# iwbn/flow-supervisor

Measured on AMD Instinct MI355X. Metric: image-pairs/s fwd+bwd, 12 GRU iters, 436x1024, higher is better.
Workload: dtype f32 (bf16x3 products); 1 GPU; RAFT full, 440x1024 (Sintel 436x1024 padded), 12 GRU iters, 4 pairs/GPU, train step = fwd + sequence loss + bwd + RCCL all-reduce + clip + AdamW; global_batch=4, parallelism=dp1, launch=hipGraph replay of the whole step

## Files before the change

### flow_supervisor_amd/_lib.py

```python
import ctypes
import functools
import os
from ctypes import POINTER, Structure, c_double, c_float, c_int, c_int64, c_void_p

import torch

_HERE = os.path.dirname(os.path.abspath(__file__))
LIB_PATH = os.environ.get("FSRAFT_LIB_PATH") or os.path.join(_HERE, "libfsraft.so")
_lib = None

c_float_p = c_void_p


class ConvDesc(Structure):
    _fields_ = [
        ("src", c_void_p * 3), ("srcC", c_int * 3), ("srcld", c_int * 3), ("nsrc", c_int),
        ("wpk", c_void_p), ("bias", c_void_p), ("wpk_split", c_void_p),
        ("B", c_int), ("H", c_int), ("W", c_int), ("KH", c_int), ("KW", c_int), ("N", c_int),
        ("dst", c_void_p * 3), ("dst_bs", c_int64 * 3), ("dst_ps", c_int64 * 3), ("dst_cs", c_int64 * 3),
        ("dst_n0", c_int * 3), ("dst_acc", c_int * 3), ("ndst", c_int),
        ("relu", c_int), ("alpha", c_float),
        ("epi", c_int),
        ("h", c_void_p), ("ldh", c_int), ("z", c_void_p), ("ldz", c_int),
        ("aux1", c_void_p), ("ld1", c_int), ("aux2", c_void_p), ("ld2", c_int), ("hid", c_int),
        ("pre", c_void_p), ("ldpre", c_int),
        ("rmask", c_void_p * 3), ("ldmask", c_int * 3), ("maskc", c_int * 3),
        ("wpk_frag", c_void_p), ("pad_h1", c_int), ("pad_w1", c_int),
        ("ws", c_void_p), ("ws_floats", c_int64),
    ]


class PackJob(Structure):
    _fields_ = [
        ("w", c_void_p * 3), ("rows", c_int * 3), ("npiece", c_int),
        ("wpk", c_void_p),
        ("cin_full", c_int), ("kh", c_int), ("kw", c_int),
        ("srcC", c_int * 3), ("srcOff", c_int * 3), ("nsrc", c_int),
        ("mode", c_int), ("flags", c_int),
        ("scale", c_float), ("accumulate", c_int),
    ]


class AugParams(Structure):
    _fields_ = [
        ("resize", c_int), ("th", c_int), ("tw", c_int),
        ("scale_x", c_float), ("scale_y", c_float),
        ("win_y", c_int), ("win_x", c_int), ("hflip", c_int), ("vflip", c_int), ("crop_y", c_int), ("crop_x", c_int),
        ("asym", c_int),
        ("brightness", c_float * 2), ("contrast", c_float * 2), ("saturation", c_float * 2), ("hue", c_float * 2),
        ("nrect", c_int),
        ("rect", (c_int * 4) * 2),
    ]


_PP = POINTER(c_void_p)
_IP = POINTER(c_int)
_S = c_void_p

SIGNATURES = {
    "fsraft_corr_build": [c_void_p, c_void_p, _PP, c_int, c_int, c_int, c_int, c_int, _S],
    "fsraft_corr_unpool_bwd": [_PP, c_int, c_int, c_int, c_int, _S],
    "fsraft_corr_lookup_fwd": [_PP, c_int, c_void_p, c_int64, c_int64, c_int64, c_void_p, c_int, c_int, c_int, c_int, c_int, _S],
    "fsraft_corr_lookup_bwd": [_PP, c_int, c_void_p, c_int64, c_int64, c_int64, c_void_p, c_int, c_int, c_int, c_int, c_int, _S],
    "fsraft_altcorr_fwd": [c_void_p, c_void_p, c_void_p, c_void_p, c_int, c_int, c_int, c_int, c_int, c_int, c_int, c_int, _S],
    "fsraft_altcorr_bwd": [c_void_p, c_void_p, c_void_p, c_void_p, c_void_p, c_void_p, c_int, c_int, c_int, c_int, c_int, c_int, c_int, c_int, _S],
    "fsraft_upsample_fwd": [c_void_p, c_int64, c_int64, c_int64, c_void_p, c_void_p, c_int, c_int, c_int, _S],
    "fsraft_upsample_bwd": [c_void_p, c_int64, c_int64, c_int64, c_void_p, c_void_p, c_void_p, c_void_p, c_void_p, c_int, c_int, c_int, _S],
    "fsraft_upflow8_fwd": [c_void_p, c_void_p, c_int, c_int, c_int, c_int, _S],
    "fsraft_upflow8_bwd": [c_void_p, c_void_p, c_int, c_int, c_int, c_int, _S],
    "fsraft_conv_ktot": [_IP, c_int, c_int, c_int],
    "fsraft_conv_forward": [POINTER(ConvDesc), _S],
    "fsraft_conv_forward_stats": [POINTER(ConvDesc), c_void_p, c_void_p, c_int, POINTER(c_int), _S],
    "fsraft_conv_wgrad": [c_void_p, c_int, c_int, _PP, _IP, _IP, c_int, c_void_p, c_void_p, c_int, c_int, c_int, c_int, c_int, _S],
    "fsraft_conv_wgrad_multi": [_PP, c_int, c_int, c_int, _PP, _IP, _IP, c_int, c_void_p, c_void_p, c_int, c_int, c_int, c_int, c_int, _S],
    "fsraft_conv_small_fwd": [c_void_p, c_int, c_int, c_void_p, c_void_p, c_void_p, c_int64, c_int64, c_int64, c_int, c_int, c_int, c_int, c_int, c_int, _S],
    "fsraft_conv_small_wgrad": [_PP, _PP, c_int, c_int, c_int, c_int, c_void_p, c_void_p, c_int, c_int, c_int, c_int, c_int, c_int, _S],
    "fsraft_conv_small_dgrad": [c_void_p, c_int, c_void_p, c_void_p, c_int, c_void_p, c_int, c_int, c_int, c_int, c_int, c_int, c_int, c_int, _S],
    "fsraft_pack_conv_weights": [POINTER(PackJob), c_int, _S],
    "fsraft_pack_conv_weight": [c_void_p, c_void_p, c_int, c_int, c_int, c_int, _IP, c_int, c_int, c_int, _S],
    "fsraft_set_rec_mfma16": [c_int],
    "fsraft_set_build_kernel": [c_int],
    "fsraft_set_dvol_policy": [c_int],
    "fsraft_set_dvol_box": [c_int],
    "fsraft_set_ktile_exact": [c_int],
    "fsraft_set_lookup_policy": [c_int],
    "fsraft_set_upsample_kernel": [c_int],
    "fsraft_conv_workspace": [c_void_p, c_int64],
    "fsraft_set_arithmetic": [c_int],
    "fsraft_get_arithmetic": [],
    "fsraft_set_tuning": [c_int, c_int],
    "fsraft_adamw_flat": [c_void_p, c_void_p, c_void_p, c_void_p, c_int64, c_void_p, c_void_p, c_float, c_void_p, c_double, c_double, c_float,
                          c_float, c_void_p, c_void_p, _S],
    "fsraft_stream_capture_id": [_S, c_void_p],
    "fsraft_stem_slots": [],
    "fsraft_stem7x7s2_fwd": [c_void_p, c_void_p, c_void_p, c_void_p, c_int, c_int, c_int, c_int, _S],
    "fsraft_stem7x7s2_wgrad": [c_void_p, c_void_p, c_void_p, c_void_p, c_int, c_int, c_int, c_int, _S],
    "fsraft_set_lookup_qb": [c_int],
    "fsraft_set_build_split": [c_int],
    "fsraft_set_gemm_split": [c_int],
    "fsraft_gemm_tn_split": [c_void_p, c_int64, c_int64, c_void_p, c_int64, c_int64, c_void_p, c_int64, c_int64, c_int, c_int, c_int, c_int, c_float, c_int, _S],
    "fsraft_gemm_f32": [c_void_p, c_int64, c_int64, c_void_p, c_int64, c_int64, c_void_p, c_int64, c_int64, c_int, c_int, c_int, c_int, c_int, c_float, c_int, _S],
    "fsraft_nchw_to_nhwc": [c_void_p, c_void_p, c_int, c_int, c_int, c_int, c_int, c_int, _S],
    "fsraft_nhwc_to_nchw": [c_void_p, c_void_p, c_int, c_int, c_int, c_int, c_int, c_int, _S],
    "fsraft_im2col7": [c_void_p, c_int64, c_int64, c_int64, c_void_p, c_int, c_int, c_int, c_int, _S],
    "fsraft_col2im7": [c_void_p, c_int, c_void_p, c_int, c_int, c_int, c_int, _S],
    "fsraft_flow_to_nhwc": [c_void_p, c_int64, c_int64, c_int64, c_void_p, c_int, c_int, c_int, c_int, _S],
    "fsraft_nhwc_to_flow": [c_void_p, c_int, c_int, c_void_p, c_int, c_int, c_int, _S],
    "fsraft_relu_bwd": [c_void_p, c_int, c_void_p, c_int, c_int64, c_int, _S],
    "fsraft_gru_bwd1": [c_void_p, c_void_p, c_void_p, c_void_p, c_void_p, c_void_p, c_int, c_void_p, c_void_p, c_void_p, c_void_p, c_int64, c_int, _S],
    "fsraft_gru_bwd2": [c_void_p, c_void_p, c_void_p, c_void_p, c_int, c_void_p, c_void_p, c_int64, c_int, _S],
    "fsraft_col_sum": [c_void_p, c_int, c_int64, c_int, c_void_p, c_float, _S],
    "fsraft_softmax_rows": [c_void_p, c_int64, c_int, _S],
    "fsraft_softmax_rows_bwd": [c_void_p, c_void_p, c_int64, c_int, _S],
    "fsraft_softmax_rows_rec": [c_void_p, c_int64, c_int, _S],
    "fsraft_softmax_rows_bwd_rec": [c_void_p, c_void_p, c_int64, c_int, _S],
    "fsraft_softmax_rows_pos": [c_void_p, c_void_p, c_int64, c_int64, c_int, c_int, c_int, c_int, c_int, _S],
    "fsraft_softmax_rows_pos_bwd": [c_void_p, c_void_p, c_void_p, c_int64, c_int64, c_int, c_int, c_int, c_int, _S],
    "fsraft_gma_mix_fwd": [c_void_p, c_int, c_void_p, c_int, c_void_p, c_void_p, c_int, c_int64, c_int, _S],
    "fsraft_gma_mix_bwd": [c_void_p, c_int, c_void_p, c_int, c_void_p, c_void_p, c_int, c_void_p, c_int, c_void_p, c_int64, c_int, _S],
    "fsraft_inorm_relu_fwd": [c_void_p, c_void_p, c_void_p, c_int64, c_int, c_float, c_int, _S],
    "fsraft_inorm_relu_bwd": [c_void_p, c_void_p, c_void_p, c_void_p, c_int64, c_int, c_int, _S],
    "fsraft_affine_relu_fwd": [c_void_p, c_void_p, c_void_p, c_void_p, c_int64, c_int, c_int, c_int, _S],
    "fsraft_affine_relu_bwd": [c_void_p, c_void_p, c_void_p, c_void_p, c_void_p, c_void_p, c_void_p, c_int64, c_int, c_int, c_int, _S],
    "fsraft_sequence_loss": [_PP, _PP, POINTER(c_float), c_int, c_int, c_void_p, c_void_p, c_float, c_float, c_int, c_int, c_int, c_void_p, _S],
    "fsraft_flow_loss_workspace_bytes": [c_int, c_int, c_int],
    "fsraft_flow_loss": [_PP, _PP, POINTER(c_float), c_int, c_int64, c_int64, c_int64, c_void_p, c_int64, c_int64, c_int64,
                         c_void_p, c_int64, c_int64, c_int, c_float, c_float, c_float, c_int, c_int, c_int,
                         c_void_p, c_void_p, c_int, c_void_p, c_void_p, c_int64, _S],
    "fsraft_corr_pool_pyramid": [_PP, c_int, c_int64, c_int, c_int, _S],
    "fsraft_corr_pool_pyramid_same": [_PP, c_int, c_int64, c_int, c_int, _S],
    "fsraft_corr_lookup_fwd_same": [_PP, c_int, c_void_p, c_int64, c_int64, c_int64, c_void_p, c_int, c_int, c_int, c_int, c_int, _S],
    "fsraft_corr_unpool_same_bwd": [_PP, c_int, c_int64, c_int, c_int, _S],
    "fsraft_corr_lookup_bwd_same": [_PP, c_int, c_void_p, c_int64, c_int64, c_int64, c_void_p, c_int, c_int, c_int, c_int, c_int, _S],
    "fsraft_corr_lookup_dcoords_same": [_PP, c_int, c_void_p, c_int64, c_int64, c_int64, c_void_p, c_int, c_void_p, c_int64, c_int64, c_int64,
                                        c_int, c_int, c_int, c_int, _S],
    "fsraft_set_norm_blocks": [c_int],
    "fsraft_get_tuning": [c_int],
    "fsraft_conv_last_route": [c_int],
    "fsraft_set_wgrad_wide": [c_int],
    "fsraft_conv_wgrad_last_tile": [],
    "fsraft_space_to_depth2": [c_void_p, c_void_p, c_int, c_int, c_int, c_int, c_int, _S],
    "fsraft_forward_interpolate": [c_void_p, c_void_p, c_int, c_int, _S],
    "fsraft_flow_metrics_scratch_bytes": [c_int, c_int, c_int],
    "fsraft_flow_metrics": [c_void_p, c_int64, c_int64, c_int64, c_void_p, c_int64, c_int64, c_int64, c_void_p, c_int64, c_int64,
                            c_int, c_int, c_int, c_void_p, c_void_p, c_void_p, c_int64, _S],
    "fsraft_flow_rad_max": [c_void_p, c_int64, c_int64, c_int64, c_int, c_int, c_int, c_float, c_void_p, _S],
    "fsraft_flow_wheel": [c_void_p, c_int64, c_int64, c_int64, c_int, c_int, c_int, c_float, c_void_p, c_float, c_int, c_void_p, _S],
    "fsraft_flow_hsv": [c_void_p, c_int64, c_int64, c_int64, c_int, c_int, c_int, c_void_p, c_float, c_int, c_void_p, _S],
    "fsraft_flow_kitti16": [c_void_p, c_int64, c_int64, c_int64, c_void_p, c_int64, c_int64, c_int, c_int, c_int, c_void_p, _S],
    "fsraft_range_map_scratch_bytes": [c_int, c_int, c_int],
    "fsraft_range_map": [c_void_p, c_int64, c_int64, c_int64, c_int, c_int, c_int, c_int, c_void_p, c_void_p, c_int64, _S],
    "fsraft_census_scratch_bytes": [c_int, c_int, c_int],
    "fsraft_census_fwd": [c_void_p, c_int64, c_int64, c_int64, c_int, c_void_p, c_int64, c_int64, c_int64, c_int, c_int, _IP,
                          c_void_p, c_int64, c_int64, c_int64, c_void_p, c_int64, c_int64, c_int, c_int, c_int,
                          c_void_p, c_void_p, c_void_p, c_void_p, c_int64, _S],
    "fsraft_census_bwd": [c_void_p, c_int64, c_int64, c_int64, c_int, c_void_p, c_int64, c_int64, c_int64, c_int, c_int, _IP,
                          c_void_p, c_int64, c_int64, c_int64, c_void_p, c_void_p, c_void_p, c_void_p, c_int, c_int, c_int,
                          c_void_p, _S],
    "fsraft_smoothness_scratch_bytes": [c_int, c_int, c_int],
    "fsraft_smoothness": [c_void_p, c_int64, c_int64, c_int64, c_int, c_int, _IP, c_void_p, c_int64, c_int64, c_int64,
                          c_int, c_int, c_int, c_int, c_float, c_int, c_void_p, c_void_p, c_void_p, c_int64, _S],
    "fsraft_fb_mask": [c_void_p, c_int64, c_int64, c_int64, c_void_p, c_int64, c_int64, c_int64, c_int, c_int, _IP,
                       c_int, c_int, c_int, c_int, c_int, c_float, c_void_p, _S],
    "fsraft_selfsup_scratch_bytes": [c_int, c_int, c_int],
    "fsraft_selfsup": [c_void_p, c_int64, c_int64, c_int64, c_int, c_int, _IP, c_void_p, c_int64, c_int64,
                       c_void_p, c_int64, c_int64, c_int64, c_void_p, c_int64, c_int64, c_int64, c_int, c_int, c_int,
                       c_int, c_float, c_void_p, c_void_p, c_void_p, c_int64, _S],
    "fsraft_augment_scratch_bytes": [c_int, c_int, c_int, c_int, c_int],
    "fsraft_augment": [c_void_p, c_void_p, c_int, c_void_p, c_void_p, c_int, c_int, c_int, POINTER(AugParams), c_int, c_int, c_int, c_int,
                       c_void_p, c_void_p, c_void_p, c_void_p, c_void_p, c_void_p, c_void_p, c_void_p, c_void_p, c_int64, _S],
    "fsraft_augment_sup_scratch_bytes": [c_int, c_int, c_int],
    "fsraft_augment_sup": [c_void_p, c_void_p, c_int, c_void_p, c_void_p, c_int, c_int, c_int, c_int, POINTER(AugParams), c_int, c_int,
                           c_void_p, c_void_p, c_void_p, c_void_p, c_void_p, c_int64, _S],
    "fsraft_inorm_relu_cl_fwd": [c_void_p, c_void_p, c_void_p, c_void_p, c_void_p, c_void_p, c_int, c_int, c_int, c_float, c_int, c_int, c_int, _S],
    "fsraft_inorm_relu_cl_bwd": [c_void_p, c_void_p, c_void_p, c_void_p, c_void_p, c_void_p, c_void_p, c_void_p, c_int, c_int, c_int,
                                 c_int, c_int, _S],
    "fsraft_affine_relu_cl_fwd": [c_void_p, c_void_p, c_void_p, c_void_p, c_void_p, c_int64, c_int, c_int, c_int, c_int, _S],
    "fsraft_affine_relu_cl_bwd": [c_void_p, c_void_p, c_void_p, c_void_p, c_void_p, c_void_p, c_void_p, c_void_p, c_void_p, c_int, c_int,
                                  c_int, c_int, c_int, _S],
    "fsraft_axpby": [c_void_p, c_void_p, c_float, c_float, c_int64, _S],
    "fsraft_sum_n": [_PP, c_int, c_void_p, c_int64, c_int, _S],
    "fsraft_bn_fold": [c_void_p, c_void_p, c_void_p, c_void_p, c_void_p, c_float, c_int, c_void_p, c_void_p, c_void_p, c_void_p, _S],
    "fsraft_bn_fold_bwd": [c_void_p, c_int, c_int, c_void_p, c_void_p, c_void_p, c_void_p, c_void_p, c_void_p, _S],
    "fsraft_bnorm_cl_fwd": [c_void_p, c_void_p, c_void_p, c_void_p, c_void_p, c_void_p, c_void_p, c_float, c_float, c_void_p, c_void_p,
                            c_void_p, c_int, c_int, c_int, c_int, c_int, _S],
    "fsraft_bnorm_cl_bwd": [c_void_p, c_void_p, c_void_p, c_void_p, c_void_p, c_void_p, c_void_p, c_void_p, c_void_p, c_int, c_int,
                            c_int, c_int, c_int, _S],
    "fsraft_vol_layout": [c_int, c_int, c_int, _IP],
    "fsraft_corr_build_tiled": [c_void_p, c_void_p, c_void_p, c_int, c_int, c_int, c_int, c_int, _S],
    "fsraft_corr_build_rec": [c_void_p, c_void_p, c_void_p, c_int, c_int, c_int, c_int, c_int, _S],
    "fsraft_corr_lookup_tiled_fwd": [c_void_p, c_int, c_void_p, c_int64, c_int64, c_int64, c_void_p, c_int, c_int, c_int, c_int, c_int, _S],
    "fsraft_corr_lookup_tiled_dcoords": [c_void_p, c_int, c_void_p, c_int64, c_int64, c_int64, c_void_p, c_void_p, c_int64, c_int64, c_int64,
                                         c_int, c_int, c_int, c_int, c_int, _S],
    "fsraft_corr_lookup_dcoords": [_PP, c_int, c_void_p, c_int64, c_int64, c_int64, c_void_p, c_int, c_void_p, c_int64, c_int64, c_int64,
                                   c_int, c_int, c_int, c_int, _S],
    "fsraft_corr_dvol_build": [_PP, _PP, POINTER(c_int64), c_int, c_void_p, c_int, c_int, c_int, c_int, c_int, c_int, c_int, c_int, c_int64,
                               c_int64, c_void_p, c_void_p, _S],
    "fsraft_set_alt_tile": [c_int],
    "fsraft_altcorr_fused_fwd": [c_void_p, _PP, c_int, c_void_p, c_int64, c_int64, c_int64, c_int, c_void_p, c_int, c_int, c_int, c_int, c_int, _S],
    "fsraft_altcorr_fused_dcoords": [c_void_p, _PP, c_int, c_void_p, c_int64, c_int64, c_int64, c_int, c_void_p, c_void_p, c_int64, c_int64,
                                     c_int64, c_int, c_int, c_int, c_int, c_int, _S],
    "fsraft_altcorr_mfma_fwd": [c_void_p, _PP, c_void_p, _PP, c_int, c_void_p, c_int64, c_int64, c_int64, c_int, c_void_p, c_int, c_int, c_int, c_int, c_int, _S],
    "fsraft_corr_f2cat": [c_void_p, c_void_p, c_int, c_int, c_int, c_int, c_int, _S],
    "fsraft_corr_dfmap2": [c_void_p, c_void_p, c_int, c_int, c_int, c_int, c_int, _S],
    "fsraft_corr_f2cat_rec": [c_void_p, c_void_p, c_int, c_int, c_int, c_int, c_int, _S],
    "fsraft_to_records": [c_void_p, c_int64, c_void_p, c_int64, c_int64, c_int, _S],
    "fsraft_gemm_rec_tn": [c_void_p, c_int64, c_int64, c_void_p, c_int64, c_int64, c_void_p, c_int64, c_int64, c_int, c_int, c_int, c_int,
                           c_float, c_int, c_int, _S],
    "fsraft_gemm_rec_nt": [c_void_p, c_int64, c_int64, c_void_p, c_int64, c_int64, c_void_p, c_int64, c_int64, c_int, c_int, c_int, c_int,
                           c_float, c_int, c_int, _S],
    "fsraft_gemm_rec_nt_list": [c_void_p, c_int64, c_int64, c_void_p, c_int64, c_int64, c_void_p, c_int64, c_int64, c_int, c_int, c_int, c_int,
                                c_float, c_int, c_int, c_void_p, c_void_p, c_int, c_int, _S],
    "fsraft_gemm_rec_tn_list": [c_void_p, c_int64, c_int64, c_void_p, c_int64, c_int64, c_void_p, c_int64, c_int64, c_int, c_int, c_int, c_int,
                                c_float, c_int, c_int, c_void_p, c_void_p, c_int, c_int, _S],
    "fsraft_corr_bwd_ktiles": [_PP, POINTER(c_int64), c_int, c_int, c_int, c_int, c_int, c_int, c_int, c_int64, c_int64, c_void_p, c_void_p,
                               c_int, c_void_p, c_void_p, c_void_p, c_int, c_void_p, _S],
}

CONV_ROUTES = {
    1: ("fwd.gemm32", "fp32"), 2: ("fwd.gemm64", "fp32"), 3: ("fwd.gemm64x128", "fp32"), 4: ("fwd.gemm128", "fp32"),
    5: ("fwd.gemm64x64", "fp32"), 6: ("fwd.gemm64x64k16", "fp32"), 7: ("fwd.gemm64x128k16", "fp32"),
    10: ("fwd.patch128x128", "bf16x3"), 11: ("fwd.patch256x128", "bf16x3"), 12: ("fwd.patch128x64", "bf16x3"),
# ... 110 lines not shown
```

### flow_supervisor_amd/core/extractor.py

```python
import os
from collections import namedtuple

import torch
import torch.nn as nn
import torch.nn.functional as F

from .. import ops
from .._lib import on_tensor_device


class _InstNormRelu(torch.autograd.Function):

    @staticmethod
    def forward(ctx, x, eps, relu):
        x = x.contiguous()
        y, stats = ops.inorm_relu_fwd(x, eps, relu)
        ctx.save_for_backward(x, stats)
        ctx.relu = relu
        return y

    @staticmethod
    def backward(ctx, g):
        x, stats = ctx.saved_tensors
        return ops.inorm_relu_bwd(g.contiguous(), x, stats, ctx.relu), None, None
# ... 309 lines not shown
STATS_IN_EPILOGUE = True
STEM_KERNEL = True
S2D_UNITS = True
TRAIN_BN = True


class _NormSums:
    __slots__ = ("acc",)

    def __init__(self):
        self.acc = None


def _conv(conv, x, bias, link=None, stem_cl=False, sums=None):
    k = conv.kernel_size
    if (_is_cl(x) and x.is_cuda and x.dtype == torch.float32 and k in ((3, 3), (1, 1)) and conv.stride == (1, 1)
            and conv.padding == (k[0] // 2, k[1] // 2) and conv.dilation == (1, 1) and conv.groups == 1
            and conv.padding_mode == "zeros" and x.shape[1] % 4 == 0 and not torch.is_autocast_enabled()):
        return _ConvCL.apply(x, conv.weight, bias, _weight_packs(conv), link, sums)
    if stem_cl and bias is None and _stem_ok(conv, x):
        return _StemFn.apply(x, conv.weight)
    return F.conv2d(_ToNCHW.apply(x) if _is_cl(x) else x, conv.weight, bias, conv.stride, conv.padding, conv.dilation, conv.groups)


_S2D_TAP = ((0, 1), (1, 0), (1, 1))


def _s2d_weight(w3):
    N, C = w3.shape[:2]
    w = w3.new_zeros(N, 2, 2, C, 2, 2)
    for ky, (ty, sy) in enumerate(_S2D_TAP):
        for kx, (tx, sx) in enumerate(_S2D_TAP):
            w[:, sy, sx, :, ty, tx] = w3[:, :, ky, kx]
    return w.reshape(N, 4 * C, 2, 2)


def _s2d_weight_grad(dw, C):
    N = dw.shape[0]
    d = dw.reshape(N, 2, 2, C, 2, 2)
    out = dw.new_empty(N, C, 3, 3)
    for ky, (ty, sy) in enumerate(_S2D_TAP):
        for kx, (tx, sx) in enumerate(_S2D_TAP):
            out[:, :, ky, kx] = d[:, sy, sx, :, ty, tx]
    return out


def _pair_structure_ok(block):
    c1 = getattr(block, "conv1", None)
    ds = block.downsample[0] if getattr(block, "downsample", None) is not None else None
    return (block.n == 2 and c1 is not None and ds is not None and c1.kernel_size == (3, 3) and c1.stride == (2, 2)
            and c1.padding == (1, 1) and c1.dilation == (1, 1) and c1.groups == 1 and ds.kernel_size == (1, 1)
            and ds.stride == (2, 2) and ds.padding == (0, 0) and ds.groups == 1)


def _pair_ok(block, C, H, W):
    return (S2D_UNITS and _pair_structure_ok(block) and H % 2 == 0 and W % 2 == 0 and C % 4 == 0
            and _cl_channels_ok(block.conv1.out_channels))


def _pair_packs(block):
    if _stale(block, "_fs_pair_packs", _pair_key(block)):
        _prepare_packs(block)
    return block.__dict__["_fs_pair_packs"]


class _StridedPairFn(torch.autograd.Function):

    @staticmethod
    def forward(ctx, x, w3, wsc, packs, pre=False):
        x = _as_cl(x)
        ctx.pre = pre
        if pre:
            B, C4, h, w = x.shape
            C, H, W = C4 // 4, 2 * h, 2 * w
            xs = x.permute(0, 2, 3, 1)
        else:
            B, C, H, W = x.shape
            h, w = H // 2, W // 2
            xs = ops.space_to_depth2(x.permute(0, 2, 3, 1))
        N, Ns = w3.shape[0], wsc.shape[0]
        y1 = torch.empty(B, h, w, N, device=x.device, dtype=torch.float32)
        ys = torch.empty(B, h, w, Ns, device=x.device, dtype=torch.float32)
        p, q = packs.conv3, packs.shortcut
        ops.conv_forward([ops.V(xs, 4 * C)], p.fwd, None, B, h, w, 2, 2, N, [ops.Dst.nhwc(y1)], wpk_split=p.fwd_split)
        ops.conv_forward([ops.V(xs, C, 0)], q.fwd, None, B, h, w, 1, 1, Ns, [ops.Dst.nhwc(ys)], wpk_split=q.fwd_split)
        ctx.save_for_backward(xs, w3, wsc)
        ctx.packs = packs
        return y1.permute(0, 3, 1, 2), ys.permute(0, 3, 1, 2)

    @staticmethod
    def backward(ctx, g1, gs):
        xs, w3, wsc = ctx.saved_tensors
        B, h, w, C4 = xs.shape
        C, N, Ns = C4 // 4, w3.shape[0], wsc.shape[0]
        p, q = ctx.packs.conv3, ctx.packs.shortcut
        g1v = ops.V(_as_cl(g1).permute(0, 2, 3, 1), N)
        gsv = ops.V(_as_cl(gs).permute(0, 2, 3, 1), Ns)
        dx = dw3 = dwsc = None
        if ctx.needs_input_grad[0]:
            dxs = torch.empty(B, h, w, C4, device=xs.device, dtype=torch.float32)
            ops.conv_forward([g1v], p.dgrad, None, B, h, w, 2, 2, C4, [ops.Dst.nhwc(dxs)], wpk_split=p.dgrad_split, pad=(0, 0))
            ops.conv_forward([gsv], q.dgrad, None, B, h, w, 1, 1, C, [ops.Dst.nhwc(dxs, 0, 0, True)], wpk_split=q.dgrad_split)
            dx = (dxs if ctx.pre else ops.space_to_depth2(dxs, inverse=True)).permute(0, 3, 1, 2)
        items = []
        if ctx.needs_input_grad[1]:
            dwpk = ops.zeros(N, ops.conv_ktot([C4], 2, 2), device=xs.device)
            ops.conv_wgrad(g1v, [ops.V(xs, C4)], dwpk, B, h, w, 2, 2)
            dw3 = torch.empty(N, C, 3, 3, device=xs.device, dtype=torch.float32)
            items.append((dwpk, [dw3], [C4], [0], C, 2, 2, 1.0, True))
        if ctx.needs_input_grad[2]:
            dwpk = ops.zeros(Ns, ops.conv_ktot([C], 1, 1), device=xs.device)
            ops.conv_wgrad(gsv, [ops.V(xs, C, 0)], dwpk, B, h, w, 1, 1)
            dwsc = torch.empty(Ns, C, 1, 1, device=xs.device, dtype=torch.float32)
            items.append((dwpk, [dwsc], [C], [0], C, 1, 1, 1.0, False))
        ops.unpack_weight_grads(items, xs.device)
        return dx, dw3, dwsc, None, None


def _norm_kind(norm):
    if isinstance(norm, nn.InstanceNorm2d) and not norm.affine and not norm.track_running_stats:
        return "instance"
    if isinstance(norm, nn.BatchNorm2d) and not norm.training and norm.track_running_stats and norm.affine:
        return "frozen_bn"
    return None


def _train_bn_ok(norm):
    return (isinstance(norm, nn.BatchNorm2d) and norm.training and norm.affine and norm.track_running_stats
            and isinstance(norm.momentum, float))


def _covered(norm):
    return _norm_kind(norm) is not None or (TRAIN_BN and _train_bn_ok(norm))


def _norm_act(norm, y, cbias, relu, res=None, link=None, sums=None, s2d=False, cl=True):
    kind = _norm_kind(norm)
    cl = cl and _cl_channels_ok(y.shape[1])
    if kind is None and cl and _covered(norm):
        return _TrainBNReluCL.apply(y, cbias, norm.weight, norm.bias, norm, relu, res, link, s2d)
    if kind is None:
        raise RuntimeError(f"no fsraft norm kernel covers {norm!r}")
    assert cl or not s2d, "space-to-depth output is a feature of the fused channels_last norm kernels"
    if kind == "instance":
        if cl:
            return _InstNormReluCL.apply(y, norm.eps, relu, res, link, sums, s2d)
        y = _InstNormRelu.apply(y, norm.eps, relu)
    else:
        bn = (y, cbias, norm.weight, norm.bias, norm.running_mean, norm.running_var, norm.eps, relu)
        if cl:
            return _FrozenBNReluCL.apply(*bn, res, link, s2d)
        y = _FrozenBNRelu.apply(*bn)
    return y if res is None else F.relu(res + y)


S2D_EMIT = True


class _S2D:
    __slots__ = ("t",)

    def __init__(self, t):
        self.t = t


def _conv_norm(conv, norm, x, relu, to_cl=False, res=None, link=None, res_link=None, s2d=False):
    kind = _norm_kind(norm)
    if kind is not None and x.is_cuda and x.dtype == torch.float32 and not torch.is_autocast_enabled():
        cl = to_cl or _is_cl(x)
        sums = _NormSums() if (kind == "instance" and cl) else None
        y = _conv(conv, x, None, link, stem_cl=to_cl, sums=sums)
        return _norm_act(norm, y, conv.bias, relu, res, res_link, sums, s2d, cl)
    if (kind is None and _covered(norm) and x.is_cuda and x.dtype == torch.float32 and not torch.is_autocast_enabled()
            and (to_cl or _is_cl(x))):
        if _cl_channels_ok(conv.out_channels):
            return _norm_act(norm, _conv(conv, x, None, link, stem_cl=to_cl), conv.bias, relu, res, res_link, None, s2d)
        assert not s2d, "space-to-depth output is a feature of the fused channels_last norm kernels"
        y = norm(_conv(conv, x, conv.bias))
        y = F.relu(y, inplace=True) if relu else y
        return y if res is None else F.relu(res + y)
    assert not s2d, "space-to-depth output is a feature of the fused channels_last norm kernels"
    if kind == "instance" and conv.bias is not None:
        y = F.conv2d(x, conv.weight, None, conv.stride, conv.padding, conv.dilation, conv.groups)
    else:
        y = conv(x)
    y = norm(y)
    y = F.relu(y, inplace=True) if relu else y
    return y if res is None else F.relu(res + y)


# ... 144 lines not shown
```

### flow_supervisor_amd/csrc/conv_common.hpp

```cpp
#pragma once
#include "gemm_core.hpp"
#include "gemm_core_split.hpp"
#include "gemm_rec.hpp"
#include <cstddef>
#include <type_traits>

struct ConvKnobs {
  int conv_tile = 0;
  int wgrad_tile = 0;
  int wgrad_blocks = 512;
  int conv_split = 1;
  int wgrad_split = 2;
  int conv_buf = 1;
  int xcd_swizzle = 0;
  int wgrad_buf = 1;
  int conv_n256 = 0;
  int wgrad_multi = 1;
  int wgrad_blocks_multi = 2048;
  int conv_uniform = 1;
  int conv_w8 = 1;
  int conv_w8_min = 64;
  int wgrad_w8 = 0;
  int wgrad_pack = 1;
  int wgrad_blocks_pack = 1024;
  int conv_n64 = 1;
  int conv_n64_min_m = 65536;
  int conv_halo = 1;
  int conv_halo_min_m = 65536;
  int wgrad_xcd = 1;
  int conv_patch = 1;
  int wgrad_patch = 1;
  int conv_patch64 = 1;
  int wgrad_patch1 = 8192;
  int conv_patch_min_m = 8192;
  int conv_ksplit = -1;
};
__attribute__((visibility("hidden"))) extern ConvKnobs knob;
__attribute__((visibility("hidden"))) extern __thread int t_route[2];

namespace {
struct Src { const float* p; int C; int ld; };
struct Dst { float* p; int64_t bs, ps, cs; int n0; int accumulate; };

struct ConvArgs {
  Src src[3]; int nsrc;
  const float* wpk; int Ktot;
  const float* bias;
  int B, H, W, KH, KW, N;
  int PH, PW;
  Dst dst[3]; int ndst;
  int relu; float alpha;
  const float* h; int ldh;
  const float* z; int ldz;
  float* aux1; int ld1;
  float* aux2; int ld2;
  int hid;
  const float* pre; int ldpre;
  const float* rmask[3]; int ldmask[3]; int maskc[3];
  float* st_sum; float* st_sq; int st_slots;
  int swz;
  int ksplit;
};

constexpr int KTAB_MAX = 512;
struct ConvArgsT {
  ConvArgs a;
  const float* ubase; int uld;
  unsigned ktab[KTAB_MAX];
};

enum { EPI_PLAIN = 0, EPI_ZR = 2, EPI_Q = 3 };

#define FS_RSRC_FLAGS 0x00020000
#define FS_OOB 0x80000000u

__device__ __forceinline__ unsigned uni(unsigned v) { return __builtin_amdgcn_readfirstlane(v); }
template <class T>
__device__ __forceinline__ const T* uni_ptr(const T* p) {
  const uint64_t u = reinterpret_cast<uint64_t>(p);
  return reinterpret_cast<const T*>((uint64_t)uni((unsigned)(u >> 32)) << 32 | uni((unsigned)u));
}
__device__ __forceinline__ __amdgpu_buffer_rsrc_t make_rsrc(const void* p, unsigned bytes) {
  const uint64_t u = reinterpret_cast<uint64_t>(p);
  const unsigned lo = __builtin_amdgcn_readfirstlane((unsigned)u), hi = __builtin_amdgcn_readfirstlane((unsigned)(u >> 32));
  void* q = reinterpret_cast<void*>((uint64_t)hi << 32 | lo);
  return __builtin_amdgcn_make_buffer_rsrc(q, 0, __builtin_amdgcn_readfirstlane(bytes), FS_RSRC_FLAGS);
}

using SWCfg128 = SplitTnCfg<128, 128, 2, 2, 2>;
using SWCfg128S = SplitTnCfg<128, 128, 2, 2, 1>;
using SWCfg128W8 = SplitTnCfg<128, 128, 2, 4, 1, 512>;
using SWCfgPack = SplitTnCfg<64, 192, 2, 2, 1>;
using SWCfgW256 = SplitTnCfg<256, 256, 2, 4, 2, 512>;
using SWCfgW128 = SplitTnCfg<128, 256, 2, 4, 2, 512>;
using Cfg128 = GemmCfg<128, 128, 32, 2, 2, 2, 2>;
using Cfg64 = GemmCfg<128, 64, 32, 4, 1, 2, 2>;
using CfgM64 = GemmCfg<64, 128, 32, 1, 4, 2, 2>;
using Cfg6464 = GemmCfg<64, 64, 32, 2, 2, 2, 2>;
using WCfg6464 = GemmCfg<64, 64, 32, 2, 2, 0, 0>;
using Cfg6464K16 = GemmCfg<64, 64, 16, 2, 2, 2, 2>;
using CfgM64K16 = GemmCfg<64, 128, 16, 1, 4, 2, 2>;

using SCfg128 = SplitCfg<128, 128, 2, 2>;
using SCfgN256 = SplitCfg<64, 256, 1, 4, 2, true>;
using SCfg256W16 = SplitCfg<256, 128, 4, 4, 2, true, 1024>;
using SCfg128W8 = SplitCfg<128, 128, 2, 4, 2, true, 512>;
using SCfg256N64 = SplitCfg<256, 64, 4, 2, 2, true, 512>;
using SCfgM64 = SplitCfg<64, 128, 1, 4, 2, true>;
using Cfg32 = GemmCfg<128, 32, 32, 4, 1, 2, 2>;
using WCfg128 = GemmCfg<128, 128, 32, 2, 2, 0, 0>;
using WCfg32 = GemmCfg<32, 128, 32, 1, 4, 0, 0>;

template <class Cfg>
constexpr int route_gemm() {
  return std::is_same_v<Cfg, Cfg32> ? 1 : std::is_same_v<Cfg, Cfg64> ? 2 : std::is_same_v<Cfg, CfgM64> ? 3 :
         std::is_same_v<Cfg, Cfg128> ? 4 : std::is_same_v<Cfg, Cfg6464> ? 5 : std::is_same_v<Cfg, Cfg6464K16> ? 6 :
         std::is_same_v<Cfg, CfgM64K16> ? 7 : 0;
}
template <class Cfg>
constexpr int route_split() {
  return std::is_same_v<Cfg, SCfgN256> ? 30 : std::is_same_v<Cfg, SCfg256N64> ? 31 : std::is_same_v<Cfg, SCfg256W16> ? 32 :
         std::is_same_v<Cfg, SCfg128W8> ? 33 : std::is_same_v<Cfg, SCfgM64> ? 34 : std::is_same_v<Cfg, SCfg128> ? 35 : 0;
}

int conv_ktot(const int* C, int nsrc, int taps) {
  int k = 0;
  for (int s = 0; s < nsrc; ++s) k += taps * (((C[s] + 31) / 32) * 32);
  return k;
}

template <class F>
void with_epi(int epi, F&& f) {
  if (epi == EPI_PLAIN) f(std::integral_constant<int, EPI_PLAIN>{});
  else if (epi == EPI_ZR) f(std::integral_constant<int, EPI_ZR>{});
  else f(std::integral_constant<int, EPI_Q>{});
}

bool fill_srcs(Src (&dst)[3], const float* const* p, const int* C, const int* ld, int nsrc) {
  for (int s = 0; s < 3; ++s) {
    dst[s] = Src{s < nsrc ? p[s] : p[0], s < nsrc ? C[s] : 0, s < nsrc ? ld[s] : 4};
    if (s < nsrc && (!p[s] || ld[s] % 4 != 0)) return false;
  }
  return true;
}

int64_t wgrad_chunk(int target, int64_t tiles, int64_t M, int words) {
  int64_t want = (target + tiles - 1) / tiles;
  if (want < 1) want = 1;
  int64_t chunk = (M + want - 1) / want;
  if (chunk < 256) chunk = 256;
  if (chunk > 32 * (words - 2)) chunk = 32 * (words - 2);
  return (chunk + 31) / 32 * 32;
// ... 4 lines not shown
```

### flow_supervisor_amd/csrc/conv_igemm.hip

```cpp
#include "conv_common.hpp"

namespace {

__device__ __forceinline__ void tile_of_block(int swz, int& bx, int& by) {
  if (!swz) return;
  const int nx = gridDim.x, T = nx * gridDim.y, i = by * nx + bx;
  const int x = i & 7, q = T >> 3, r = T & 7;
  const int t = x * q + (x < r ? x : r) + (i >> 3);
  bx = t % nx; by = t / nx;
}

template <class Cfg>
struct ConvALoader {
  static constexpr int BM = Cfg::BM, BK = Cfg::BK, LD = Cfg::LDA;
  static constexpr int F4 = BK / 4;
  static constexpr int NF4 = BM * F4 / 256;
  static constexpr int NREG = NF4 * 4;
  static constexpr int NCH = NF4;
  const float* p0; const float* p1; const float* p2;
  int C0, C1, C2, ld0, ld1, ld2;
  int cpt0, cpt1, cpt2;
  int taps, KW, PH, PW, H, W;
  int py[NF4], px[NF4];
  int64_t pb[NF4];
  __device__ __forceinline__ bool fetch_chunk(int kt, float (&r)[NREG], int j) const {
    const int n0 = taps * cpt0, n1 = taps * cpt1;
    const bool is1 = kt >= n0, is2 = kt >= n0 + n1;
    const int k = kt - (is1 ? n0 : 0) - (is2 ? n1 : 0);
    const int C = C0 + (is1 ? C1 - C0 : 0) + (is2 ? C2 - C1 : 0);
    const int ld = ld0 + (is1 ? ld1 - ld0 : 0) + (is2 ? ld2 - ld1 : 0);
    const int cpt = cpt0 + (is1 ? cpt1 - cpt0 : 0) + (is2 ? cpt2 - cpt1 : 0);
    const float* p = p0 + (is1 ? p1 - p0 : 0) + (is2 ? p2 - p1 : 0);
    const int tap = k / cpt, c0 = (k % cpt) * BK;
    const int dy = tap / KW - PH, dx = tap % KW - PW;
    const int kq = (threadIdx.x + 256 * j) % F4;
    const int yy = py[j] + dy, xx = px[j] + dx, c = c0 + kq * 4;
    const bool ok = py[j] >= 0 && yy >= 0 && yy < H && xx >= 0 && xx < W && c < C;
    const f32x4 v = gload4(p + (ok ? (pb[j] + (int64_t)yy * W + xx) * ld + c : 0));
    r[4 * j + 0] = v[0]; r[4 * j + 1] = v[1]; r[4 * j + 2] = v[2]; r[4 * j + 3] = v[3];
    return ok;
  }
  __device__ __forceinline__ void store_chunk(float* t, const float (&r)[NREG], int j, bool ok) const {
    const int e = threadIdx.x + 256 * j;
    const int row = e / F4, kq = e % F4;
#pragma unroll
    for (int c = 0; c < 4; ++c) t[(kq * 4 + c) * LD + row] = ok ? r[4 * j + c] : 0.f;
  }
};

template <class Cfg>
struct SplitConvALoader {
  static constexpr int NCH = Cfg::NCH_A, NREG = NCH * 4;
  const float* p0; const float* p1; const float* p2;
  int C0, C1, C2, ld0, ld1, ld2, cpt0, cpt1, cpt2;
  int taps, KW, PH, PW, H, W;
  int py[NCH], px[NCH];
  int pofs[NCH];
  __device__ __forceinline__ void fetch_chunk(int kt, float (&r)[NREG], int j) const {
    const int n0 = taps * cpt0, n1 = taps * cpt1;
    const bool is1 = kt >= n0, is2 = kt >= n0 + n1;
    const int k = kt - (is1 ? n0 : 0) - (is2 ? n1 : 0);
    const int C = C0 + (is1 ? C1 - C0 : 0) + (is2 ? C2 - C1 : 0);
    const int ld = ld0 + (is1 ? ld1 - ld0 : 0) + (is2 ? ld2 - ld1 : 0);
    const int cpt = cpt0 + (is1 ? cpt1 - cpt0 : 0) + (is2 ? cpt2 - cpt1 : 0);
    const float* p = p0 + (is1 ? p1 - p0 : 0) + (is2 ? p2 - p1 : 0);
    const int tap = k / cpt, c0 = (k % cpt) * 32;
    const int dy = tap / KW - PH, dx = tap % KW - PW;
    const int kq = (threadIdx.x + 256 * j) & 7;
    const int c = c0 + kq * 4;
    const bool ok = ((unsigned)(py[j] + dy) < (unsigned)H) && ((unsigned)(px[j] + dx) < (unsigned)W) && c < C;
    const float* src = ok ? p + (int64_t)(pofs[j] + dy * W + dx) * ld + c : g_fsraft_zero16;
    const f32x4 v = gload4(src);
    r[4 * j + 0] = v[0]; r[4 * j + 1] = v[1]; r[4 * j + 2] = v[2]; r[4 * j + 3] = v[3];
  }
  __device__ __forceinline__ void stage_chunk(char* tile, const float* r4, int j) const {
    stage_convert<Cfg::PITCH>(tile, threadIdx.x + 256 * j, r4);
  }
};

template <class Cfg>
struct BufConvALoader {
  static constexpr int NCH = Cfg::NCH_A, NREG = NCH * 4;
  const float* b0; const float* b1; const float* b2; unsigned nb0, nb1, nb2;
  unsigned ld0x4, ld1x4, ld2x4;
  const unsigned __attribute__((address_space(4)))* ktab;
  unsigned tapmask[NCH];
  unsigned pofs[NCH];
  unsigned kq16;
  __device__ __forceinline__ void fetch_tile(int kt, float (&r)[NREG]) const {
    const unsigned e = ktab[__builtin_amdgcn_readfirstlane(kt)];
    const unsigned soff = (e & 0xffffu) << 4, tap = (e >> 16) & 15u, src = (e >> 20) & 3u, crem = (e >> 22) & 63u;
    const bool s1 = src >= 1, s2 = src >= 2;
    const unsigned ldb = ld0x4 + (s1 ? ld1x4 - ld0x4 : 0u) + (s2 ? ld2x4 - ld1x4 : 0u);
    const float* bp = b0 + (s1 ? b1 - b0 : 0) + (s2 ? b2 - b1 : 0);
    const __amdgpu_buffer_rsrc_t rs = make_rsrc(bp, 0x7fffffffu);
    const unsigned cok = kq16 < crem * 4u ? 1u : 0u;
#pragma unroll
    for (int j = 0; j < NCH; ++j) {
      const unsigned bad = (__builtin_amdgcn_ubfe(tapmask[j], tap, 1u) & cok) ^ 1u;
      const unsigned voff = (bad << 31) | (__umul24(pofs[j], ldb) + kq16);
      const u32x4 v = __builtin_amdgcn_raw_buffer_load_b128(rs, voff, soff, 0);
      const f32x4 f = __builtin_bit_cast(f32x4, v);
      r[4 * j + 0] = f[0]; r[4 * j + 1] = f[1]; r[4 * j + 2] = f[2]; r[4 * j + 3] = f[3];
    }
  }
  __device__ __forceinline__ void stage_chunk(char* tile, const float* r4, int j) const {
    stage_convert<Cfg::PITCH>(tile, threadIdx.x + Cfg::NT * j, r4);
  }
};

template <class Cfg>
struct BufConvALoaderU {
  static constexpr int NCH = Cfg::NCH_A, NREG = NCH * 4;
  const float* base;
  const unsigned __attribute__((address_space(4)))* ktab;
  unsigned tapmask[NCH];
  unsigned voff0[NCH];
  unsigned kq16;
  __device__ __forceinline__ void fetch_tile(int kt, float (&r)[NREG]) const {
    const int ku = __builtin_amdgcn_readfirstlane(kt);
    const unsigned soff = ktab[2 * ku], e = ktab[2 * ku + 1];
    const unsigned tap = e & 15u, crem4 = (e >> 4) * 4u;
    const __amdgpu_buffer_rsrc_t rs = make_rsrc(base, 0x7fffffffu);
    const unsigned cok = kq16 < crem4 ? 1u : 0u;
#pragma unroll
    for (int j = 0; j < NCH; ++j) {
      const unsigned bad = (__builtin_amdgcn_ubfe(tapmask[j], tap, 1u) & cok) ^ 1u;
      const u32x4 v = __builtin_amdgcn_raw_buffer_load_b128(rs, (bad << 31) | voff0[j], soff, 0);
      const f32x4 f = __builtin_bit_cast(f32x4, v);
      r[4 * j + 0] = f[0]; r[4 * j + 1] = f[1]; r[4 * j + 2] = f[2]; r[4 * j + 3] = f[3];
    }
  }
  __device__ __forceinline__ void stage_chunk(char* tile, const float* r4, int j) const {
    stage_convert<Cfg::PITCH>(tile, threadIdx.x + Cfg::NT * j, r4);
  }
};

template <class Cfg>
struct BufWeightLoader {
  static constexpr int NCH = Cfg::NCH_B, NREG = NCH * 4;
  const char* base; unsigned nbytes;
  unsigned voff[NCH];
  __device__ __forceinline__ void fetch_tile(int kt, float (&r)[NREG]) const {
    const int ku = __builtin_amdgcn_readfirstlane(kt);
    const __amdgpu_buffer_rsrc_t rs = make_rsrc(base, ku < 0 ? 0u : nbytes);
    const unsigned soff = ku < 0 ? 0u : (unsigned)ku * 128u;
#pragma unroll
    for (int j = 0; j < NCH; ++j) {
      const u32x4 v = __builtin_amdgcn_raw_buffer_load_b128(rs, voff[j], soff, 0);
      const f32x4 f = __builtin_bit_cast(f32x4, v);
      r[4 * j + 0] = f[0]; r[4 * j + 1] = f[1]; r[4 * j + 2] = f[2]; r[4 * j + 3] = f[3];
    }
  }
  __device__ __forceinline__ void stage_chunk(char* tile, const float* r4, int j) const {
    stage_copy<Cfg::PITCH>(tile, threadIdx.x + Cfg::NT * j, r4);
  }
};

template <class Cfg>
struct SplitWeightLoader {
  static constexpr int NCH = Cfg::NCH_B, NREG = NCH * 4;
  const char* base;
  int64_t row_bytes;
  int rows_valid;
  __device__ __forceinline__ void fetch_chunk(int kt, float (&r)[NREG], int j) const {
    const int e = threadIdx.x + 256 * j;
    const int row = e >> 3, part = e & 7;
    const char* src = (row < rows_valid && kt >= 0) ? base + row * row_bytes + (int64_t)kt * 128 + part * 16
                                                    : reinterpret_cast<const char*>(g_fsraft_zero16);
    const f32x4 v = gload4(src);
    r[4 * j + 0] = v[0]; r[4 * j + 1] = v[1]; r[4 * j + 2] = v[2]; r[4 * j + 3] = v[3];
  }
  __device__ __forceinline__ void stage_chunk(char* tile, const float* r4, int j) const {
    stage_copy<Cfg::PITCH>(tile, threadIdx.x + 256 * j, r4);
  }
};

template <class Cfg, int EPI>
__device__ __forceinline__ void conv_epilogue(const ConvArgs& a, f32x16 (&acc)[Cfg::TM][Cfg::TN], int m0, int n0) {
  const int HW = a.H * a.W;
  const int M = a.B * HW;
  const int lane = threadIdx.x & 63, wave = threadIdx.x >> 6;
#pragma unroll
  for (int nt = 0; nt < Cfg::TN; ++nt) {
    const int n = n0 + acc_col<Cfg>(nt);
    const bool nok = n < a.N;
    const float bias = (nok && a.bias) ? a.bias[n] : 0.f;
    int di = 0;
    if (a.ndst > 1 && n >= a.dst[1].n0) di = 1;
    if (a.ndst > 2 && n >= a.dst[2].n0) di = 2;
    float* dp = di == 0 ? a.dst[0].p : di == 1 ? a.dst[1].p : a.dst[2].p;
    const int64_t dbs = di == 0 ? a.dst[0].bs : di == 1 ? a.dst[1].bs : a.dst[2].bs;
    const int64_t dps = di == 0 ? a.dst[0].ps : di == 1 ? a.dst[1].ps : a.dst[2].ps;
    const int64_t dcs = di == 0 ? a.dst[0].cs : di == 1 ? a.dst[1].cs : a.dst[2].cs;
    const int dn0 = di == 0 ? a.dst[0].n0 : di == 1 ? a.dst[1].n0 : a.dst[2].n0;
    const bool dacc = (di == 0 ? a.dst[0].accumulate : di == 1 ? a.dst[1].accumulate : a.dst[2].accumulate) != 0;
    const float* mk = di == 0 ? a.rmask[0] : di == 1 ? a.rmask[1] : a.rmask[2];
    const int ldm = di == 0 ? a.ldmask[0] : di == 1 ? a.ldmask[1] : a.ldmask[2];
    const int mkc = di == 0 ? a.maskc[0] : di == 1 ? a.maskc[1] : a.maskc[2];
#pragma unroll
    for (int mt = 0; mt < Cfg::TM; ++mt) {
      const int mbase = m0 + (wave / Cfg::WN) * (Cfg::TM * 32) + mt * 32 + 4 * (lane >> 5);
      const int b0 = mbase / HW, pix0 = mbase - b0 * HW;
      if (EPI == EPI_PLAIN) {
#pragma unroll
        for (int hb = 0; hb < 2; ++hb) {
          int off[8];
#pragma unroll
          for (int q = 0; q < 8; ++q) {
            const int r = hb * 8 + q;
            const int d = (r & 3) + 8 * (r >> 2);
            int pix = pix0 + d, b = b0;
            if (pix >= HW) { pix -= HW; ++b; }
            const bool ok = nok && (mbase + d < M);
            off[q] = ok ? (int)(b * dbs + pix * dps + (n - dn0) * dcs) : -1;
          }
          float old[8];
#pragma unroll
          for (int q = 0; q < 8; ++q) old[q] = (dacc && off[q] >= 0) ? dp[off[q]] : 0.f;
#pragma unroll
          for (int q = 0; q < 8; ++q) {
            float v = (acc[mt][nt][hb * 8 + q] + bias) * a.alpha;
            if (a.relu) v = fmaxf(v, 0.f);
            v += old[q];
            if (off[q] >= 0 && mk && n - dn0 < mkc) {
              const int r = hb * 8 + q;
              const int64_t m = mbase + (r & 3) + 8 * (r >> 2);
              if (mk[m * ldm + (n - dn0)] <= 0.f) v = 0.f;
            }
// ... 168 lines not shown
      if (isz) {
        *reinterpret_cast<f32x4*>(a.dst[0].p + m * a.dst[0].ps + c) = v;
      } else {
        *reinterpret_cast<f32x4*>(a.aux2 + m * a.ld2 + c) = v;
        f32x4 rh;
#pragma unroll
        for (int i = 0; i < 4; ++i) rh[i] = v[i] * hh[i];
        *reinterpret_cast<f32x4*>(a.aux1 + m * a.ld1 + c) = rh;
      }
    }
  } else {
#pragma unroll 4
    for (int row = rsub; row < Cfg::BM; row += RPP) {
      const int64_t m = row_m(row);
      if (m < 0) { if (PATCH) continue; else break; }
      f32x4 v = *reinterpret_cast<const f32x4*>(tile + row * LD + c4 * 4);
      if (a.pre) v += gload4(a.pre + m * a.ldpre + n);
      const f32x4 hh = gload4(a.h + m * a.ldh + n);
      const f32x4 zz = gload4(a.z + m * a.ldz + n);
      f32x4 hn;
#pragma unroll
      for (int i = 0; i < 4; ++i) {
        v[i] = tanhf(v[i]);
        hn[i] = (1.f - zz[i]) * hh[i] + zz[i] * v[i];
      }
      *reinterpret_cast<f32x4*>(a.aux1 + m * a.ld1 + n) = v;
      *reinterpret_cast<f32x4*>(a.dst[0].p + m * a.dst[0].ps + n) = hn;
    }
  }
}

__device__ __forceinline__ bool epilogue_rows_ok(const ConvArgs& a) {
  bool ok = true;
  for (int i = 0; i < a.ndst; ++i)
    ok = ok && a.dst[i].cs == 1 && (a.dst[i].ps & 3) == 0 && (a.dst[i].n0 & 3) == 0 && ((uintptr_t)a.dst[i].p & 15) == 0 &&
         a.dst[i].bs == a.dst[i].ps * (int64_t)(a.H * a.W);
  return ok;
}

bool epilogue_rows_ok_host(const ConvArgs& a) {
  bool ok = true;
  for (int i = 0; i < a.ndst; ++i)
    ok = ok && a.dst[i].cs == 1 && (a.dst[i].ps & 3) == 0 && (a.dst[i].n0 & 3) == 0 && ((uintptr_t)a.dst[i].p & 15) == 0 &&
         a.dst[i].bs == a.dst[i].ps * (int64_t)(a.H * a.W);
  return ok;
}

template <class Cfg, int EPI>
__global__ __launch_bounds__(256) void conv_igemm_kernel(ConvArgs a) {
  __shared__ __attribute__((aligned(16))) float lds[Cfg::LDS_FLOATS];
  const int HW = a.H * a.W;
  const int M = a.B * HW;
  const int n0 = blockIdx.x * Cfg::BN, m0 = blockIdx.y * Cfg::BM;
  ConvALoader<Cfg> la;
  la.p0 = a.src[0].p; la.C0 = a.src[0].C; la.ld0 = a.src[0].ld; la.cpt0 = (a.src[0].C + 31) / 32 * (32 / Cfg::BK);
  la.p1 = a.src[1].p; la.C1 = a.src[1].C; la.ld1 = a.src[1].ld; la.cpt1 = a.nsrc > 1 ? (a.src[1].C + 31) / 32 * (32 / Cfg::BK) : 0;
  la.p2 = a.src[2].p; la.C2 = a.src[2].C; la.ld2 = a.src[2].ld; la.cpt2 = a.nsrc > 2 ? (a.src[2].C + 31) / 32 * (32 / Cfg::BK) : 0;
  if (a.nsrc < 2) { la.p1 = a.src[0].p; la.C1 = 0; la.ld1 = 4; la.cpt1 = 1; }
  if (a.nsrc < 3) { la.p2 = a.src[0].p; la.C2 = 0; la.ld2 = 4; la.cpt2 = 1; }
  la.taps = a.KH * a.KW; la.KW = a.KW; la.PH = a.PH; la.PW = a.PW; la.H = a.H; la.W = a.W;
#pragma unroll
  for (int j = 0; j < ConvALoader<Cfg>::NF4; ++j) {
    const int row = (threadIdx.x + 256 * j) / ConvALoader<Cfg>::F4;
    const int m = m0 + row;
    if (m < M) {
      const int b = m / HW, pix = m % HW;
      la.py[j] = pix / a.W; la.px[j] = pix % a.W; la.pb[j] = (int64_t)b * HW;
    } else {
      la.py[j] = -1; la.px[j] = 0; la.pb[j] = 0;
    }
  }
  RowMajorTileLoader<Cfg::BN, Cfg::BK, Cfg::LDB> lb{a.wpk + (int64_t)n0 * a.Ktot, a.Ktot, a.N - n0, a.Ktot};
  f32x16 acc[Cfg::TM][Cfg::TN];
#pragma unroll
  for (int i = 0; i < Cfg::TM; ++i)
#pragma unroll
    for (int j = 0; j < Cfg::TN; ++j)
#pragma unroll
      for (int r = 0; r < 16; ++r) acc[i][j][r] = 0.f;
  gemm_mainloop<Cfg>(lds, a.Ktot / Cfg::BK, la, lb, acc);
  conv_epilogue<Cfg, EPI>(a, acc, m0, n0);
}

template <class Cfg, int EPI, int BUF = 0>
__global__ __launch_bounds__(Cfg::NT) void conv_igemm_split_kernel(const std::conditional_t<BUF != 0, ConvArgsT, ConvArgs> args) {
  static_assert(Cfg::NT == 256 || BUF != 0, "wider workgroups use the buffer-addressed loaders");
  __shared__ __attribute__((aligned(16))) char lds[Cfg::LDS_ALLOC];
  const ConvArgs& a = [&]() -> const ConvArgs& { if constexpr (BUF != 0) return args.a; else return args; }();
  const int HW = a.H * a.W;
  const int M = a.B * HW;
  int bx = blockIdx.x, by = blockIdx.y;
  tile_of_block(a.swz, bx, by);
  const int n0 = bx * Cfg::BN, m0 = by * Cfg::BM;
  f32x16 acc[Cfg::TM][Cfg::TN];
#pragma unroll
  for (int i = 0; i < Cfg::TM; ++i)
#pragma unroll
    for (int j = 0; j < Cfg::TN; ++j)
#pragma unroll
      for (int r = 0; r < 16; ++r) acc[i][j][r] = 0.f;
  if constexpr (BUF != 0) {
    const int PH = a.PH, PW = a.PW, taps = a.KH * a.KW;
    const auto* ktab = (const unsigned __attribute__((address_space(4)))*)(
        (const char __attribute__((address_space(4)))*)__builtin_amdgcn_kernarg_segment_ptr() + offsetof(ConvArgsT, ktab));
    int kt0 = 0, KTs = a.Ktot / 32;
    if (a.ksplit > 1) {
      const int per = (KTs + a.ksplit - 1) / a.ksplit;
      kt0 = (int)blockIdx.z * per;
      KTs = min(per, KTs - kt0);
      ktab += kt0 * (BUF >= 2 ? 2 : 1);
    }
    unsigned tapmask[Cfg::NCH_A], pofs[Cfg::NCH_A];
#pragma unroll
    for (int j = 0; j < Cfg::NCH_A; ++j) {
      const int m = m0 + ((threadIdx.x + Cfg::NT * j) >> 3);
      unsigned mask = 0;
      if (m < M) {
        const int pix = m % HW, y = pix / a.W, x = pix % a.W;
        for (int t = 0; t < taps; ++t) {
          const int yy = y + t / a.KW - PH, xx = x + t % a.KW - PW;
          if ((unsigned)yy < (unsigned)a.H && (unsigned)xx < (unsigned)a.W) mask |= 1u << t;
        }
      }
      tapmask[j] = mask; pofs[j] = m < M ? m : 0;
    }
    BufWeightLoader<Cfg> lb;
    lb.base = uni_ptr(reinterpret_cast<const char*>(a.wpk) + (int64_t)n0 * a.Ktot * 4 + (int64_t)kt0 * 128);
    lb.nbytes = 0x7fffffffu;
#pragma unroll
    for (int j = 0; j < BufWeightLoader<Cfg>::NCH; ++j) {
      const int e = threadIdx.x + Cfg::NT * j;
      lb.voff[j] = (e >> 3) < a.N - n0 ? (unsigned)((e >> 3) * a.Ktot * 4 + (e & 7) * 16) : FS_OOB;
    }
    if constexpr (BUF >= 2) {
      BufConvALoaderU<Cfg> la;
      la.base = uni_ptr(args.ubase); la.ktab = ktab; la.kq16 = (threadIdx.x & 7) * 16;
      const unsigned ldb = uni((unsigned)args.uld * 4u);
#pragma unroll
      for (int j = 0; j < Cfg::NCH_A; ++j) { la.tapmask[j] = tapmask[j]; la.voff0[j] = pofs[j] * ldb + la.kq16; }
      split_mainloop<Cfg, BufConvALoaderU<Cfg>, BufWeightLoader<Cfg>, true>(lds, KTs, la, lb, acc);
    } else {
      BufConvALoader<Cfg> la;
      la.ld0x4 = uni(a.src[0].ld * 4); la.ld1x4 = uni(a.src[1].ld * 4); la.ld2x4 = uni(a.src[2].ld * 4);
      la.b0 = uni_ptr(a.src[0].p - (int64_t)(PH * a.W + PW) * a.src[0].ld); la.nb0 = 0x7fffffffu;
      la.b1 = uni_ptr(a.src[1].p - (int64_t)(PH * a.W + PW) * a.src[1].ld); la.nb1 = 0x7fffffffu;
      la.b2 = uni_ptr(a.src[2].p - (int64_t)(PH * a.W + PW) * a.src[2].ld); la.nb2 = 0x7fffffffu;
      la.ktab = ktab;
      la.kq16 = (threadIdx.x & 7) * 16;
#pragma unroll
      for (int j = 0; j < Cfg::NCH_A; ++j) { la.tapmask[j] = tapmask[j]; la.pofs[j] = pofs[j]; }
      split_mainloop<Cfg, BufConvALoader<Cfg>, BufWeightLoader<Cfg>, true>(lds, KTs, la, lb, acc);
    }
    if constexpr (EPI == EPI_PLAIN && Cfg::LDS_ALLOC >= Cfg::BM * (Cfg::BN + 4) * 4) {
      if (a.ksplit > 1) {
        conv_epilogue_lds<Cfg, EPI_PLAIN>(a, acc, m0, n0, reinterpret_cast<float*>(lds), true, 0, 0, 0, (int64_t)blockIdx.z * M);
        return;
      }
    }
  } else {
  SplitConvALoader<Cfg> la;
  la.p0 = a.src[0].p; la.C0 = a.src[0].C; la.ld0 = a.src[0].ld; la.cpt0 = (a.src[0].C + 31) / 32;
  la.p1 = a.src[1].p; la.C1 = a.src[1].C; la.ld1 = a.src[1].ld; la.cpt1 = a.nsrc > 1 ? (a.src[1].C + 31) / 32 : 0;
  la.p2 = a.src[2].p; la.C2 = a.src[2].C; la.ld2 = a.src[2].ld; la.cpt2 = a.nsrc > 2 ? (a.src[2].C + 31) / 32 : 0;
  if (a.nsrc < 2) { la.p1 = a.src[0].p; la.C1 = 0; la.ld1 = 4; la.cpt1 = 1; }
  if (a.nsrc < 3) { la.p2 = a.src[0].p; la.C2 = 0; la.ld2 = 4; la.cpt2 = 1; }
  la.taps = a.KH * a.KW; la.KW = a.KW; la.PH = a.PH; la.PW = a.PW; la.H = a.H; la.W = a.W;
#pragma unroll
  for (int j = 0; j < SplitConvALoader<Cfg>::NCH; ++j) {
    const int m = m0 + ((threadIdx.x + 256 * j) >> 3);
    if (m < M) {
      const int pix = m % HW;
      la.py[j] = pix / a.W; la.px[j] = pix % a.W; la.pofs[j] = m;
    } else {
      la.py[j] = -(1 << 20); la.px[j] = 0; la.pofs[j] = 0;
    }
  }
  SplitWeightLoader<Cfg> lb{reinterpret_cast<const char*>(a.wpk) + (int64_t)n0 * a.Ktot * 4, (int64_t)a.Ktot * 4, a.N - n0};
  split_mainloop<Cfg>(lds, a.Ktot / 32, la, lb, acc);
  }
  if constexpr (Cfg::LDS_ALLOC >= Cfg::BM * (Cfg::BN + 4) * 4) {
    if (EPI != EPI_PLAIN || epilogue_rows_ok(a)) {
      conv_epilogue_lds<Cfg, EPI>(a, acc, m0, n0, reinterpret_cast<float*>(lds));
      return;
    }
  }
  conv_epilogue<Cfg, EPI>(a, acc, m0, n0);
}

constexpr int HALO_TH = 4, HALO_TW = 32, HALO_PW = HALO_TW + 2, HALO_ROWS = (HALO_TH + 2) * HALO_PW;
struct HaloArgs {
  const float* x; int ldx, C;
  const char* wpk;
  const float* bias;
  float* out; int64_t obs, ops;
  int N, B, H, W, relu;
  int acc;
  float* st_sum; float* st_sq; int st_slots;
};

template <int CG, int TN>
__global__ __launch_bounds__(256) void conv3x3_halo_kernel(const HaloArgs a) {
  constexpr int PLANE = HALO_ROWS * 128;
  constexpr int NCHH = (HALO_ROWS * CG * 8 + 255) / 256, KT = 9 * CG;
  __shared__ __attribute__((aligned(16))) char lds[CG * PLANE];
  const int lane = threadIdx.x & 63, wave = threadIdx.x >> 6;
  const int wm = wave >> 1, wn = wave & 1, l31 = lane & 31, lh = lane >> 5;
  const int x0 = blockIdx.x * HALO_TW, y0 = blockIdx.y * HALO_TH, b = blockIdx.z;

  const int NB = (a.N + 31) >> 5;
  const char* wbase = uni_ptr(a.wpk);
  struct BFrag { u32x4 v[TN][4]; };
  auto fetch_b = [&](int kt, BFrag& f) {
    const int ku = __builtin_amdgcn_readfirstlane(kt < KT ? kt : KT - 1);
    const __amdgpu_buffer_rsrc_t rs = make_rsrc(wbase, 0x7fffffffu);
#pragma unroll
    for (int nt = 0; nt < TN; ++nt) {
      const int nb = wn * TN + nt;
      const unsigned soff = (unsigned)((ku * NB + (nb < NB ? nb : 0)) * 4096);
      const unsigned voff = nb < NB ? (unsigned)lane * 16u : FS_OOB;
#pragma unroll
      for (int q = 0; q < 4; ++q) f.v[nt][q] = __builtin_amdgcn_raw_buffer_load_b128(rs, voff, soff + 1024u * q, 0);
    }
  };
  BFrag f[4];
  fetch_b(0, f[0]);
  fetch_b(1, f[1]);
  fetch_b(2, f[2]);

  {
    const float* img = uni_ptr(a.x + (int64_t)b * a.H * a.W * a.ldx);
    const __amdgpu_buffer_rsrc_t rs = make_rsrc(img, 0x7fffffffu);
    float rh[NCHH * 4];
#pragma unroll
    for (int j = 0; j < NCHH; ++j) {
// ... 40 lines not shown
      for (int mt = 0; mt < 2; ++mt)
#pragma unroll
        for (int nt = 0; nt < TN; ++nt) {
          const bf16x8 bh = __builtin_bit_cast(bf16x8, f.v[nt][s]), bl = __builtin_bit_cast(bf16x8, f.v[nt][2 + s]);
          acc[mt][nt] = __builtin_amdgcn_mfma_f32_32x32x16_bf16(al[mt], bh, acc[mt][nt], 0, 0, 0);
          acc[mt][nt] = __builtin_amdgcn_mfma_f32_32x32x16_bf16(ah[mt], bl, acc[mt][nt], 0, 0, 0);
          acc[mt][nt] = __builtin_amdgcn_mfma_f32_32x32x16_bf16(ah[mt], bh, acc[mt][nt], 0, 0, 0);
        }
    }
  };
  for (int kt = 0; kt < KT; kt += 4) {
#pragma unroll
    for (int i = 0; i < 4; ++i)
      if (kt + i < KT) {
        fetch_b(kt + i + 3, f[(i + 3) & 3]);
        compute(kt + i, f[i]);
      }
  }

  if (a.st_sum) {
    __syncthreads();
    float* red = reinterpret_cast<float*>(lds);
#pragma unroll
    for (int nt = 0; nt < TN; ++nt) {
      float s1 = 0.f, s2 = 0.f;
#pragma unroll
      for (int mt = 0; mt < 2; ++mt) {
        const int py = y0 + 2 * wm + mt;
#pragma unroll
        for (int r = 0; r < 16; ++r) {
          const int px = x0 + (r & 3) + 8 * (r >> 2) + 4 * lh;
          const float v = (py < a.H && px < a.W) ? acc[mt][nt][r] : 0.f;
          s1 += v; s2 += v * v;
        }
      }
      s1 += __shfl_xor(s1, 32, 64); s2 += __shfl_xor(s2, 32, 64);
      const int col = wn * (32 * TN) + nt * 32 + l31;
      if (lh == 0) { red[(wm * 2 + 0) * (64 * TN) + col] = s1; red[(wm * 2 + 1) * (64 * TN) + col] = s2; }
    }
    __syncthreads();
    if ((int)threadIdx.x < 64 * TN && (int)threadIdx.x < a.N) {
      const int col = threadIdx.x;
      const int slot = (int)((blockIdx.y * gridDim.x + blockIdx.x) % (unsigned)a.st_slots);
      const int64_t o = ((int64_t)b * a.st_slots + slot) * a.N + col;
      atomicAdd(a.st_sum + o, red[col] + red[2 * (64 * TN) + col]);
      atomicAdd(a.st_sq + o, red[(64 * TN) + col] + red[3 * (64 * TN) + col]);
    }
  }
  float* outb = a.out + (int64_t)b * a.obs;
#pragma unroll
  for (int mt = 0; mt < 2; ++mt) {
    const int py = y0 + 2 * wm + mt;
    if (py >= a.H) continue;
#pragma unroll
    for (int nt = 0; nt < TN; ++nt) {
      const int n = wn * (32 * TN) + nt * 32 + l31;
      if (n >= a.N) continue;
      const float bv = a.bias ? a.bias[n] : 0.f;
      float old[16];
#pragma unroll
      for (int r = 0; r < 16; ++r) {
        const int px = x0 + (r & 3) + 8 * (r >> 2) + 4 * lh, pc = px < a.W ? px : a.W - 1;
        old[r] = a.acc ? outb[(int64_t)(py * a.W + pc) * a.ops + n] : 0.f;
      }
#pragma unroll
      for (int r = 0; r < 16; ++r) {
        const int px = x0 + (r & 3) + 8 * (r >> 2) + 4 * lh;
        if (px >= a.W) continue;
        float v = acc[mt][nt][r] + bv;
        if (a.relu) v = fmaxf(v, 0.f);
        outb[(int64_t)(py * a.W + px) * a.ops + n] = v + old[r];
      }
    }
  }
}

template <int CG, int TN>
int launch_halo(const HaloArgs& h, hipStream_t s) {
  dim3 grid(ceil_div(h.W, HALO_TW), ceil_div(h.H, HALO_TH), h.B);
  hipLaunchKernelGGL((conv3x3_halo_kernel<CG, TN>), grid, dim3(256), 0, s, h);
  return fs_launch_status();
}

bool build_ktab(const ConvArgs& a, ConvArgsT& t) {
  const int taps = a.KH * a.KW, KT = a.Ktot / 32;
  const int64_t M = (int64_t)a.B * a.H * a.W;
  if (KT > KTAB_MAX || taps > 15) return false;
  int kt = 0;
  for (int s = 0; s < a.nsrc; ++s) {
    const int C = a.src[s].C, ld = a.src[s].ld, cpt = (C + 31) / 32;
    if (M * ld * 4 >= (int64_t)FS_OOB) return false;
    for (int i = 0; i < taps * cpt; ++i, ++kt) {
        const int tap = i / cpt, c = i % cpt;
        const int64_t soff = ((int64_t)((tap / a.KW) * a.W + tap % a.KW) * ld + c * 32) * 4;
        if (soff % 16 != 0 || soff / 16 > 0xffff) return false;
        const int crem = C - c * 32 < 32 ? C - c * 32 : 32;
        t.ktab[kt] = (unsigned)(soff / 16) | (unsigned)tap << 16 | (unsigned)s << 20 | (unsigned)crem << 22;
      }
  }
  if (kt != KT) return false;
  t.a = a;
  return true;
}

bool build_ktab_uniform(const ConvArgs& a, ConvArgsT& t) {
  const int taps = a.KH * a.KW, KT = a.Ktot / 32, PH = a.PH, PW = a.PW;
  const int64_t M = (int64_t)a.B * a.H * a.W;
  if (!knob.conv_uniform || 2 * KT > KTAB_MAX || taps > 15) return false;
  const int ld = a.src[0].ld;
  const float* lo = a.src[0].p;
  for (int s = 0; s < a.nsrc; ++s) {
    if (a.src[s].ld != ld) return false;
    if (a.src[s].p < lo) lo = a.src[s].p;
  }
  const float* base = lo - (int64_t)(PH * a.W + PW) * ld;
  int kt = 0;
  for (int s = 0; s < a.nsrc; ++s) {
    const int C = a.src[s].C, cpt = (C + 31) / 32;
    const int64_t delta = (a.src[s].p - lo) * 4;
    for (int tap = 0; tap < taps; ++tap)
      for (int c = 0; c < cpt; ++c, ++kt) {
        const int64_t soff = delta + ((int64_t)((tap / a.KW) * a.W + tap % a.KW) * ld + c * 32) * 4;
        if (soff + M * ld * 4 + 256 >= (int64_t)FS_OOB) return false;
        const int crem = C - c * 32 < 32 ? C - c * 32 : 32;
        t.ktab[2 * kt] = (unsigned)soff;
        t.ktab[2 * kt + 1] = (unsigned)tap | (unsigned)crem << 4;
      }
  }
  if (kt != KT) return false;
  t.a = a; t.ubase = base; t.uld = ld;
  return true;
}


template <int EPI>
__global__ __launch_bounds__(256) void conv_finish_kernel(const ConvArgs a, const float* __restrict__ ws, int S, int ldw) {
  const int HW = a.H * a.W;
  const int64_t M = (int64_t)a.B * HW;
  const int C4 = (a.N + 3) / 4;
  for (int64_t e = (int64_t)blockIdx.x * 256 + threadIdx.x; e < M * C4; e += (int64_t)gridDim.x * 256) {
    const int64_t m = e / C4;
    const int n = (int)(e % C4) * 4;
    const int nv = a.N - n < 4 ? a.N - n : 4;
    f32x4 v = {0.f, 0.f, 0.f, 0.f};
    if (a.bias) {
#pragma unroll
      for (int i = 0; i < 4; ++i) v[i] = i < nv ? a.bias[n + i] : 0.f;
    }
    for (int s = 0; s < S; ++s) {
      const f32x4 p = gload4(ws + ((int64_t)s * M + m) * ldw + n);
#pragma unroll
      for (int i = 0; i < 4; ++i) v[i] += p[i];
    }
    if (EPI == EPI_PLAIN) {
      int di = 0;
      if (a.ndst > 1 && n >= a.dst[1].n0) di = 1;
      if (a.ndst > 2 && n >= a.dst[2].n0) di = 2;
      float* dp = di == 0 ? a.dst[0].p : di == 1 ? a.dst[1].p : a.dst[2].p;
      const int64_t dbs = di == 0 ? a.dst[0].bs : di == 1 ? a.dst[1].bs : a.dst[2].bs;
      const int64_t dps = di == 0 ? a.dst[0].ps : di == 1 ? a.dst[1].ps : a.dst[2].ps;
      const int64_t dcs = di == 0 ? a.dst[0].cs : di == 1 ? a.dst[1].cs : a.dst[2].cs;
      const int dn0 = di == 0 ? a.dst[0].n0 : di == 1 ? a.dst[1].n0 : a.dst[2].n0;
      const bool dacc = (di == 0 ? a.dst[0].accumulate : di == 1 ? a.dst[1].accumulate : a.dst[2].accumulate) != 0;
      const float* mk = di == 0 ? a.rmask[0] : di == 1 ? a.rmask[1] : a.rmask[2];
      const int ldm = di == 0 ? a.ldmask[0] : di == 1 ? a.ldmask[1] : a.ldmask[2];
      const int mkc = di == 0 ? a.maskc[0] : di == 1 ? a.maskc[1] : a.maskc[2];
      const int64_t b = m / HW, pix = m - b * HW;
      float* o = dp + b * dbs + pix * dps + (int64_t)(n - dn0) * dcs;
      for (int i = 0; i < nv; ++i) {
        float r = v[i] * a.alpha;
        if (a.relu) r = fmaxf(r, 0.f);
        if (dacc) r += o[i * dcs];
        if (mk && n - dn0 + i < mkc && mk[m * ldm + (n - dn0) + i] <= 0.f) r = 0.f;
        o[i * dcs] = r;
      }
    } else if (EPI == EPI_ZR) {
      const bool isz = n < a.hid;
      const int c = isz ? n : n - a.hid;
      if (a.pre) v += gload4(a.pre + m * a.ldpre + n);
#pragma unroll
      for (int i = 0; i < 4; ++i) v[i] = 1.0f / (1.0f + expf(-v[i]));
      if (isz) {
        *reinterpret_cast<f32x4*>(a.dst[0].p + m * a.dst[0].ps + c) = v;
      } else {
        const f32x4 hh = gload4(a.h + m * a.ldh + c);
        *reinterpret_cast<f32x4*>(a.aux2 + m * a.ld2 + c) = v;
        f32x4 rh;
#pragma unroll
        for (int i = 0; i < 4; ++i) rh[i] = v[i] * hh[i];
        *reinterpret_cast<f32x4*>(a.aux1 + m * a.ld1 + c) = rh;
      }
    } else {
      if (a.pre) v += gload4(a.pre + m * a.ldpre + n);
      const f32x4 hh = gload4(a.h + m * a.ldh + n);
      const f32x4 zz = gload4(a.z + m * a.ldz + n);
      f32x4 hn;
#pragma unroll
      for (int i = 0; i < 4; ++i) {
        v[i] = tanhf(v[i]);
        hn[i] = (1.f - zz[i]) * hh[i] + zz[i] * v[i];
      }
      *reinterpret_cast<f32x4*>(a.aux1 + m * a.ld1 + n) = v;
      *reinterpret_cast<f32x4*>(a.dst[0].p + m * a.dst[0].ps + n) = hn;
    }
  }
}

thread_local float* t_reg_ws = nullptr;
thread_local int64_t t_reg_ws_floats = 0;
thread_local float* g_conv_ws = nullptr;
thread_local int64_t g_conv_ws_floats = 0;

int pick_ksplit(int64_t tiles, int KT, int N, int64_t M, int ldw, int bm) {
  int S = 1;
  if (knob.conv_ksplit >= 2) S = knob.conv_ksplit;
  else if (knob.conv_ksplit == -1 && bm == 64 && tiles <= 150 && N <= 256 && KT >= 16) S = (int)((400 + tiles - 1) / tiles);
  else if (knob.conv_ksplit == -1 && bm == 128 && tiles <= 120 && N <= 256 && KT >= (N <= 128 ? 36 : 48)) S = tiles <= 115 ? (int)(230 / tiles) : 2;
  if (S > KT / 6) S = KT / 6;
  if (S > 6) S = 6;
  while (S > 1 && (int64_t)S * M * ldw > g_conv_ws_floats) --S;
  if (S > 1) {
    const int per = (KT + S - 1) / S;
    S = (KT + per - 1) / per;
  }
  return S < 2 ? 1 : S;
}

template <class Cfg>
int launch_conv_split(const ConvArgs& a, int epi, hipStream_t s) {
  const int M = a.B * a.H * a.W;
  dim3 grid(ceil_div(a.N, Cfg::BN), ceil_div(M, Cfg::BM));
  ConvArgsT t;
  const int swz = knob.xcd_swizzle || (grid.x >= 2 && (int64_t)grid.x * grid.y >= 2048);
  const bool buf = knob.conv_buf == 2 || (knob.conv_buf == 1 && Cfg::BM == 64) || Cfg::BN == 256 || Cfg::NT != 256;
  if constexpr (Cfg::LDS_ALLOC >= Cfg::BM * (Cfg::BN + 4) * 4) {
    const int ldw = (a.N + 3) / 4 * 4;
    const bool gru_ok = epi == EPI_PLAIN || (a.N % 4 == 0 && (!a.pre || a.ldpre % 4 == 0));
    const int S = (buf && g_conv_ws && gru_ok && (Cfg::BM == 64 || (Cfg::BM == 128 && Cfg::NT == 512) || knob.conv_ksplit >= 2)) ? pick_ksplit((int64_t)grid.x * grid.y, a.Ktot / 32, a.N, M, ldw, Cfg::BM) : 1;
    if (S > 1) {
      const bool uni_tab = build_ktab_uniform(a, t);
      if (uni_tab || build_ktab(a, t)) {
        ConvArgs& p = t.a;
        p.swz = 0;
        p.ksplit = S;
        p.dst[0] = Dst{g_conv_ws, (int64_t)a.H * a.W * ldw, ldw, 1, 0, 0};
        p.dst[1] = p.dst[2] = p.dst[0];
        p.ndst = 1; p.bias = nullptr; p.relu = 0; p.alpha = 1.0f;
        for (int i = 0; i < 3; ++i) p.rmask[i] = nullptr;
        dim3 g3(grid.x, grid.y, S);
        t_route[0] = route_split<Cfg>() + 100;
        if (uni_tab) hipLaunchKernelGGL((conv_igemm_split_kernel<Cfg, EPI_PLAIN, 2>), g3, dim3(Cfg::NT), 0, s, t);
        else hipLaunchKernelGGL((conv_igemm_split_kernel<Cfg, EPI_PLAIN, 1>), g3, dim3(Cfg::NT), 0, s, t);
        int rc = fs_launch_status();
        if (rc) return rc;
        const int64_t work = (int64_t)M * (ldw / 4);
        const int fb = (int)((work + 255) / 256 < 4096 ? (work + 255) / 256 : 4096);
        with_epi(epi, [&](auto e) { hipLaunchKernelGGL(conv_finish_kernel<decltype(e)::value>, dim3(fb), dim3(256), 0, s, a, g_conv_ws, S, ldw); });
        return fs_launch_status();
      }
    }
  }
  if (buf && build_ktab_uniform(a, t)) {
    t.a.swz = swz;
    t_route[0] = route_split<Cfg>();
    with_epi(epi, [&](auto e) { hipLaunchKernelGGL((conv_igemm_split_kernel<Cfg, decltype(e)::value, 2>), grid, dim3(Cfg::NT), 0, s, t); });
    return fs_launch_status();
  }
  if (buf && build_ktab(a, t)) {
    t.a.swz = swz;
    t_route[0] = route_split<Cfg>();
    with_epi(epi, [&](auto e) { hipLaunchKernelGGL((conv_igemm_split_kernel<Cfg, decltype(e)::value, 1>), grid, dim3(Cfg::NT), 0, s, t); });
    return fs_launch_status();
  }
  if constexpr (Cfg::NT != 256) {
    return -1;
  } else {
  t_route[0] = route_split<Cfg>();
  with_epi(epi, [&](auto e) { hipLaunchKernelGGL((conv_igemm_split_kernel<Cfg, decltype(e)::value>), grid, dim3(256), 0, s, a); });
  return fs_launch_status();
  }
}

template <class Cfg>
int launch_conv_split_plain(const ConvArgs& a, hipStream_t s) {
  const int M = a.B * a.H * a.W;
  dim3 grid(ceil_div(a.N, Cfg::BN), ceil_div(M, Cfg::BM));
  ConvArgsT t;
  if (build_ktab_uniform(a, t)) {
    t_route[0] = route_split<Cfg>();
    hipLaunchKernelGGL((conv_igemm_split_kernel<Cfg, EPI_PLAIN, 2>), grid, dim3(Cfg::NT), 0, s, t);
    return fs_launch_status();
  }
  if (build_ktab(a, t)) {
    t_route[0] = route_split<Cfg>();
    hipLaunchKernelGGL((conv_igemm_split_kernel<Cfg, EPI_PLAIN, 1>), grid, dim3(Cfg::NT), 0, s, t);
    return fs_launch_status();
  }
  return -1;
}

template <class Cfg>
int launch_conv(const ConvArgs& a, int epi, hipStream_t s) {
  const int M = a.B * a.H * a.W;
  dim3 grid(ceil_div(a.N, Cfg::BN), ceil_div(M, Cfg::BM));
  t_route[0] = route_gemm<Cfg>();
  with_epi(epi, [&](auto e) { hipLaunchKernelGGL((conv_igemm_kernel<Cfg, decltype(e)::value>), grid, dim3(256), 0, s, a); });
  return fs_launch_status();
}

#include "conv_patch.inc"

}

extern "C" int fsraft_conv_ktot(const int* srcC, int nsrc, int KH, int KW) {
  if (!srcC || nsrc < 1 || nsrc > 3) return -1;
  return conv_ktot(srcC, nsrc, KH * KW);
}

namespace {
struct StatReq { float* sum; float* sq; int slots; bool done; };
thread_local StatReq t_stat{nullptr, nullptr, 0, false};
template <class Args>
void attach_stats(Args& p, bool want) {
  if (want) { p.st_sum = t_stat.sum; p.st_sq = t_stat.sq; p.st_slots = t_stat.slots; }
}
}

extern "C" int fsraft_conv_forward(const fsraft_conv_desc* d, hipStream_t stream) {
  if (!d || d->nsrc < 1 || d->nsrc > 3 || d->ndst < 1 || d->ndst > 3 || !d->wpk || d->N < 1) return FS_ERR_ARG;
  const bool want_stats = t_stat.sum != nullptr && d->epi == EPI_PLAIN && d->ndst == 1 && !d->relu && d->alpha == 1.0f && !d->dst_acc[0] &&
                          !d->rmask[0] && !d->bias && d->dst_n0[0] == 0 && d->N % 4 == 0;
  if (d->ws && (((uintptr_t)d->ws & 15) || d->ws_floats < 0)) return FS_ERR_ARG;
  t_route[0] = 0;
  g_conv_ws = d->ws ? d->ws : t_reg_ws;
  g_conv_ws_floats = d->ws ? d->ws_floats : t_reg_ws_floats;
  ConvArgs a{};
  if (!fill_srcs(a.src, d->src, d->srcC, d->srcld, d->nsrc)) return FS_ERR_ARG;
  for (int s = 0; s < d->nsrc; ++s) if (d->srcC[s] < 1) return FS_ERR_ARG;
  a.nsrc = d->nsrc;
  a.wpk = d->wpk; a.Ktot = conv_ktot(d->srcC, d->nsrc, d->KH * d->KW); a.bias = d->bias;
  a.B = d->B; a.H = d->H; a.W = d->W; a.KH = d->KH; a.KW = d->KW; a.N = d->N;
  a.PH = d->pad_h1 ? d->pad_h1 - 1 : d->KH / 2; a.PW = d->pad_w1 ? d->pad_w1 - 1 : d->KW / 2;
  if (a.PH < 0 || a.PH >= d->KH || a.PW < 0 || a.PW >= d->KW) return FS_ERR_ARG;
  for (int i = 0; i < 3; ++i) {
    const int j = i < d->ndst ? i : 0;
    a.dst[i] = Dst{d->dst[j], d->dst_bs[j], d->dst_ps[j], d->dst_cs[j], d->dst_n0[j], d->dst_acc[j]};
    if (i < d->ndst && !d->dst[i]) return FS_ERR_ARG;
  }
  a.ndst = d->ndst; a.relu = d->relu; a.alpha = d->alpha;
  a.h = d->h; a.ldh = d->ldh; a.z = d->z; a.ldz = d->ldz; a.aux1 = d->aux1; a.ld1 = d->ld1; a.aux2 = d->aux2; a.ld2 = d->ld2;
  a.hid = d->hid;
  a.pre = d->epi == EPI_PLAIN ? nullptr : d->pre; a.ldpre = d->ldpre;
  if (a.pre && (d->ldpre % 4 != 0 || ((uintptr_t)d->pre & 15))) return FS_ERR_ARG;
  for (int i = 0; i < 3; ++i) {
    const bool on = d->epi == EPI_PLAIN && i < d->ndst && d->rmask[i] != nullptr;
    a.rmask[i] = on ? d->rmask[i] : nullptr; a.ldmask[i] = d->ldmask[i]; a.maskc[i] = d->maskc[i];
    if (on && (d->ldmask[i] % 4 != 0 || ((uintptr_t)d->rmask[i] & 15))) return FS_ERR_ARG;
  }
  a.swz = knob.xcd_swizzle;
  if (d->epi == EPI_ZR && (!d->h || !d->aux1 || !d->aux2 || d->hid * 2 != d->N)) return FS_ERR_ARG;
  if (d->epi == EPI_Q && (!d->h || !d->z || !d->aux1)) return FS_ERR_ARG;
  if (d->epi != EPI_PLAIN && d->epi != EPI_ZR && d->epi != EPI_Q) return FS_ERR_ARG;
  if (knob.conv_patch && knob.conv_patch64 && knob.conv_split == 1 && d->wpk_split && d->epi == EPI_PLAIN && d->KH == 3 && d->KW == 3 &&
      d->N > 32 && d->N <= 64 && (int64_t)d->B * d->H * d->W >= knob.conv_patch_min_m) {
    ConvArgs p = a;
    p.wpk = d->wpk_split;
    attach_stats(p, want_stats);
    const int rc = launch_conv_patch(p, d->epi, stream);
    if (rc >= 0) { t_stat.done = want_stats; return rc; }
  }
  if (knob.conv_halo && knob.conv_split == 1 && d->wpk_frag && d->epi == EPI_PLAIN && d->nsrc == 1 && d->KH == 3 && d->KW == 3 &&
      a.PH == 1 && a.PW == 1 &&
      d->srcC[0] % 4 == 0 && d->srcC[0] > 32 && d->srcC[0] <= 64 && d->N <= 128 && d->N > 32 && d->ndst == 1 &&
      d->dst_cs[0] == 1 && d->dst_n0[0] == 0 && !(d->dst_acc[0] && d->relu) && !a.rmask[0] && d->alpha == 1.0f &&
      (int64_t)d->B * d->H * d->W >= knob.conv_halo_min_m && (int64_t)d->H * d->W * d->srcld[0] * 4 < 0x7fffffff) {
    HaloArgs h{d->src[0], d->srcld[0], d->srcC[0], reinterpret_cast<const char*>(d->wpk_frag), d->bias,
               d->dst[0], d->dst_bs[0], d->dst_ps[0], d->N, d->B, d->H, d->W, d->relu, d->dst_acc[0], nullptr, nullptr, 0};
    attach_stats(h, want_stats);
    t_stat.done = want_stats;
    t_route[0] = d->N > 64 ? 21 : 20;
    return d->N > 64 ? launch_halo<2, 2>(h, stream) : launch_halo<2, 1>(h, stream);
  }
  if (d->N <= 32 && d->epi == EPI_PLAIN) return launch_conv<Cfg32>(a, d->epi, stream);
  if (d->N <= 64 && d->epi == EPI_PLAIN && !(knob.conv_split && d->wpk_split && knob.conv_buf)) return launch_conv<Cfg64>(a, d->epi, stream);
  const int M = d->B * d->H * d->W;
  if (knob.conv_split && d->wpk_split && d->N > 32) {
    a.wpk = d->wpk_split;
    const bool narrow = knob.conv_buf != 0 || (int64_t)ceil_div(d->N, 128) * ceil_div(M, 128) < 400;
    if (knob.conv_patch && knob.conv_split == 1 && d->KH * d->KW > 1 && d->N > 64 && M >= knob.conv_patch_min_m) {
      ConvArgs p = a;
      attach_stats(p, want_stats);
      const int rc = launch_conv_patch(p, d->epi, stream);
      if (rc >= 0) { t_stat.done = want_stats; return rc; }
    }
    if (knob.conv_split == 5 || (knob.conv_split == 1 && knob.conv_n256 && d->N >= 256 &&
                              ceil_div(d->N, 256) * 256 <= ceil_div(d->N, 128) * 128))
      return launch_conv_split<SCfgN256>(a, d->epi, stream);
    if (knob.conv_split == 1 && knob.conv_n64 && d->N <= 64 && d->epi == EPI_PLAIN && M >= knob.conv_n64_min_m) {
      const int rc = launch_conv_split_plain<SCfg256N64>(a, stream);
      if (rc >= 0) return rc;
    }
    if (knob.conv_split == 1 && ((knob.conv_w8 == 1 && d->N >= 192 && d->N <= 512 && M >= 16384) || knob.conv_w8 == 2) && d->N >= 192) {
      const int rc = launch_conv_split<SCfg256W16>(a, d->epi, stream);
      if (rc >= 0) return rc;
    }
    if (knob.conv_w8 && knob.conv_split == 1 && (int64_t)ceil_div(d->N, 128) * ceil_div(M, 128) >= knob.conv_w8_min) {
      const int rc = launch_conv_split<SCfg128W8>(a, d->epi, stream);
      if (rc >= 0) return rc;
    }
    if (knob.conv_split == 3) return launch_conv_split<SCfgM64>(a, d->epi, stream);
    if (knob.conv_split == 4) return launch_conv_split<SCfg128>(a, d->epi, stream);
    return narrow ? launch_conv_split<SCfgM64>(a, d->epi, stream) : launch_conv_split<SCfg128>(a, d->epi, stream);
  }
  if (knob.conv_tile == 3) return launch_conv<Cfg6464>(a, d->epi, stream);
  if (knob.conv_tile == 4) return launch_conv<Cfg6464K16>(a, d->epi, stream);
  if (knob.conv_tile == 5) return launch_conv<CfgM64K16>(a, d->epi, stream);
  if (knob.conv_tile == 2) return launch_conv<CfgM64>(a, d->epi, stream);
  if (knob.conv_tile == 1) return launch_conv<Cfg128>(a, d->epi, stream);
  if ((int64_t)ceil_div(d->N, 128) * ceil_div(M, 128) < 512) return launch_conv<CfgM64>(a, d->epi, stream);
  return launch_conv<Cfg128>(a, d->epi, stream);
}

extern "C" int fsraft_conv_forward_stats(const fsraft_conv_desc* d, float* sum, float* sq, int slots, int* done, hipStream_t stream) {
  if (!sum || !sq || slots < 1 || !done) return FS_ERR_ARG;
  t_stat = StatReq{sum, sq, slots, false};
  const int rc = fsraft_conv_forward(d, stream);
  *done = (rc == FS_OK && t_stat.done) ? 1 : 0;
  t_stat = StatReq{nullptr, nullptr, 0, false};
  return rc;
}


extern "C" int fsraft_conv_workspace(float* ws, int64_t floats) {
  if (ws && (((uintptr_t)ws & 15) || floats < 0)) return FS_ERR_ARG;
  t_reg_ws = ws;
  t_reg_ws_floats = ws ? floats : 0;
  return FS_OK;
}
```

### flow_supervisor_amd/csrc/conv_tuning.hip

```cpp
#include "conv_common.hpp"
#include <climits>

ConvKnobs knob;
__thread int t_route[2] = {0, 0};

namespace {
const struct { int key; int ConvKnobs::*member; } KNOB_TABLE[] = {
    {FSRAFT_KEY_CONV_TILE, &ConvKnobs::conv_tile},
    {FSRAFT_KEY_WGRAD_TILE, &ConvKnobs::wgrad_tile},
    {FSRAFT_KEY_WGRAD_BLOCKS, &ConvKnobs::wgrad_blocks},
    {FSRAFT_KEY_CONV_ARITH, &ConvKnobs::conv_split},
    {FSRAFT_KEY_WGRAD_ARITH, &ConvKnobs::wgrad_split},
    {FSRAFT_KEY_CONV_BUF, &ConvKnobs::conv_buf},
    {FSRAFT_KEY_XCD_SWIZZLE, &ConvKnobs::xcd_swizzle},
    {FSRAFT_KEY_WGRAD_BUF, &ConvKnobs::wgrad_buf},
    {FSRAFT_KEY_CONV_N256, &ConvKnobs::conv_n256},
    {FSRAFT_KEY_WGRAD_MULTI, &ConvKnobs::wgrad_multi},
    {FSRAFT_KEY_WGRAD_BLOCKS_MULTI, &ConvKnobs::wgrad_blocks_multi},
    {FSRAFT_KEY_CONV_UNIFORM, &ConvKnobs::conv_uniform},
    {FSRAFT_KEY_CONV_W8, &ConvKnobs::conv_w8},
    {FSRAFT_KEY_CONV_W8_MIN, &ConvKnobs::conv_w8_min},
    {FSRAFT_KEY_WGRAD_W8, &ConvKnobs::wgrad_w8},
    {FSRAFT_KEY_WGRAD_PACK, &ConvKnobs::wgrad_pack},
    {FSRAFT_KEY_WGRAD_BLOCKS_PACK, &ConvKnobs::wgrad_blocks_pack},
    {FSRAFT_KEY_CONV_N64, &ConvKnobs::conv_n64},
    {FSRAFT_KEY_CONV_N64_MIN_M, &ConvKnobs::conv_n64_min_m},
    {FSRAFT_KEY_CONV_HALO, &ConvKnobs::conv_halo},
    {FSRAFT_KEY_CONV_HALO_MIN_M, &ConvKnobs::conv_halo_min_m},
    {FSRAFT_KEY_WGRAD_XCD, &ConvKnobs::wgrad_xcd},
    {FSRAFT_KEY_CONV_PATCH, &ConvKnobs::conv_patch},
    {FSRAFT_KEY_WGRAD_PATCH, &ConvKnobs::wgrad_patch},
    {FSRAFT_KEY_CONV_PATCH64, &ConvKnobs::conv_patch64},
    {FSRAFT_KEY_WGRAD_PATCH1, &ConvKnobs::wgrad_patch1},
    {FSRAFT_KEY_CONV_PATCH_MIN_M, &ConvKnobs::conv_patch_min_m},
    {FSRAFT_KEY_CONV_KSPLIT, &ConvKnobs::conv_ksplit},
};

int* knob_of(int key) {
  for (const auto& e : KNOB_TABLE)
    if (e.key == key) return &(knob.*e.member);
  return nullptr;
}
}

extern "C" int fsraft_set_tuning(int key, int value) {
  int* k = knob_of(key);
  if (!k) return FS_ERR_ARG;
  *k = value;
  return FS_OK;
}

extern "C" int fsraft_get_tuning(int key) {
  const int* k = knob_of(key);
  return k ? *k : INT_MIN;
}

extern "C" int fsraft_conv_last_route(int which) {
  return which == 0 || which == 1 ? t_route[which] : -1;
}

extern "C" int fsraft_set_arithmetic(int mode) {
  if (mode != 0 && mode != 1) return FS_ERR_ARG;
  knob.conv_split = mode ? 1 : 0;
  knob.wgrad_split = mode ? 2 : 0;
  fsraft_set_build_split(mode);
  fsraft_set_gemm_split(mode);
  return FS_OK;
}
extern "C" int fsraft_get_arithmetic(void) { return knob.conv_split != 0 ? 1 : 0; }
```

### flow_supervisor_amd/csrc/conv_wgrad.hip

```cpp
#include "conv_common.hpp"

namespace {

struct WgradArgs {
  const float* dy; int ldy; int Cout;
  Src src[3]; int nsrc;
  float* dwpk; int Ktot;
  int B, H, W, KH, KW;
  int kchunk;
  float* dbias;
  int xcd_xt, xcd_yt, xcd_groups;
  int bx0, by0;
};

constexpr int WGRAD_MAX_SEG = 16;
struct WgradArgsM {
  WgradArgs a;
  int nseg, zs;
  const float* dys[WGRAD_MAX_SEG];
  const float* srcs[3][WGRAD_MAX_SEG];
};

template <class Cfg>
struct ShiftedXLoader {
  static constexpr int BN = Cfg::BN, BK = Cfg::BK, LD = Cfg::LDB;
  static constexpr int F4 = BN / 4;
  static constexpr int NF4 = BK * F4 / 256;
  static constexpr int NREG = NF4 * 4;
  static constexpr int NCH = NF4;
  const float* p; int ld, cvalid;
  int dy, dx, H, W, HW; int64_t M; int64_t m_begin, m_end;
  __device__ __forceinline__ bool fetch_chunk(int kt, float (&r)[NREG], int j) const {
    const int e = threadIdx.x + 256 * j;
    const int k = e / F4, c4 = e % F4;
    const int64_t m = m_begin + (int64_t)kt * BK + k;
    const int64_t mm = m < m_end ? m : m_begin;
    const int64_t b = mm / HW; const int pix = (int)(mm % HW);
    const int yy = pix / W + dy, xx = pix % W + dx;
    const bool ok = m < m_end && c4 * 4 < cvalid && yy >= 0 && yy < H && xx >= 0 && xx < W;
    const f32x4 v = gload4(p + (ok ? (b * HW + (int64_t)yy * W + xx) * ld + c4 * 4 : 0));
    r[4 * j + 0] = v[0]; r[4 * j + 1] = v[1]; r[4 * j + 2] = v[2]; r[4 * j + 3] = v[3];
    return ok;
  }
  __device__ __forceinline__ void store_chunk(float* t, const float (&r)[NREG], int j, bool ok) const {
    const int e = threadIdx.x + 256 * j;
    const int k = e / F4, c4 = e % F4;
    f32x4 v = {r[4 * j + 0], r[4 * j + 1], r[4 * j + 2], r[4 * j + 3]};
    const f32x4 z = {0.f, 0.f, 0.f, 0.f};
    *reinterpret_cast<f32x4*>(t + k * LD + c4 * 4) = ok ? v : z;
  }
};

template <class Cfg>
struct DyLoader {
  static constexpr int BM = Cfg::BM, BK = Cfg::BK, LD = Cfg::LDA;
  static constexpr int F4 = BM / 4;
  static constexpr int NF4 = BK * F4 / 256;
  static constexpr int NREG = NF4 * 4;
  static_assert((BK * F4) % 256 == 0, "dy tile must divide over 256 threads");
  static constexpr int NCH = NF4;
  const float* p; int ld, cvalid; int64_t m_begin, m_end;
  __device__ __forceinline__ bool fetch_chunk(int kt, float (&r)[NREG], int j) const {
    const int e = threadIdx.x + 256 * j;
    const int k = e / F4, c4 = e % F4;
    const int64_t m = m_begin + (int64_t)kt * BK + k;
    const bool ok = m < m_end && c4 * 4 < cvalid;
    const f32x4 v = gload4(p + (ok ? m * ld + c4 * 4 : 0));
    r[4 * j + 0] = v[0]; r[4 * j + 1] = v[1]; r[4 * j + 2] = v[2]; r[4 * j + 3] = v[3];
    return ok;
  }
  __device__ __forceinline__ void store_chunk(float* t, const float (&r)[NREG], int j, bool ok) const {
    const int e = threadIdx.x + 256 * j;
    const int k = e / F4, c4 = e % F4;
    f32x4 v = {r[4 * j + 0], r[4 * j + 1], r[4 * j + 2], r[4 * j + 3]};
    const f32x4 z = {0.f, 0.f, 0.f, 0.f};
    *reinterpret_cast<f32x4*>(t + k * LD + c4 * 4) = ok ? v : z;
  }
};

template <class Cfg>
struct SplitDyLoader {
  static constexpr int NCH = Cfg::NCH_A, NREG = NCH * 4;
  const float* p; int ld, cvalid; int64_t m_begin, m_end;
  __device__ __forceinline__ void fetch_chunk(int kt, float (&r)[NREG], int j) const {
    const int e = threadIdx.x + 256 * j;
    const int k = e / (Cfg::BM / 4), c4 = e % (Cfg::BM / 4);
    const int64_t m = m_begin + (int64_t)kt * 32 + k;
    const bool ok = m < m_end && c4 * 4 < cvalid;
    const f32x4 v = gload4(ok ? p + m * ld + c4 * 4 : g_fsraft_zero16);
    r[4 * j + 0] = v[0]; r[4 * j + 1] = v[1]; r[4 * j + 2] = v[2]; r[4 * j + 3] = v[3];
  }
};
template <class Cfg>
struct SplitShiftedXLoader {
  static constexpr int NCH = Cfg::NCH_B, NREG = NCH * 4;
  const float* p; int ld, cvalid;
  int dy, dx, H, W, HW; int64_t m_begin, m_end;
  __device__ __forceinline__ void fetch_chunk(int kt, float (&r)[NREG], int j) const {
    const int e = threadIdx.x + 256 * j;
    const int k = e / (Cfg::BN / 4), c4 = e % (Cfg::BN / 4);
    const int64_t m = m_begin + (int64_t)kt * 32 + k;
    const int64_t mm = m < m_end ? m : m_begin;
    const int pix = (int)(mm % HW);
    const int yy = pix / W + dy, xx = pix % W + dx;
    const bool ok = m < m_end && c4 * 4 < cvalid && (unsigned)yy < (unsigned)H && (unsigned)xx < (unsigned)W;
    const f32x4 v = gload4(ok ? p + (mm + dy * W + dx) * ld + c4 * 4 : g_fsraft_zero16);
    r[4 * j + 0] = v[0]; r[4 * j + 1] = v[1]; r[4 * j + 2] = v[2]; r[4 * j + 3] = v[3];
  }
};

constexpr int WGRAD_MASK_WORDS = 2048;
template <class Cfg>
struct BufDyLoader {
  static constexpr int NCH = Cfg::NCH_A, NREG = NCH * 4;
  const float* base; unsigned ld4; int npix;
  unsigned voff[NCH]; int krow[NCH];
  __device__ __forceinline__ void fetch_tile(int kt, float (&r)[NREG]) const {
    const int ku = __builtin_amdgcn_readfirstlane(kt);
    const __amdgpu_buffer_rsrc_t rs = make_rsrc(base, 0x7fffffffu);
    const unsigned soff = (unsigned)ku * 32u * ld4;
    const int left = npix - ku * 32;
#pragma unroll
    for (int j = 0; j < NCH; ++j) {
      const unsigned voffj = voff[j] | (krow[j] < left ? 0u : FS_OOB);
      const u32x4 v = __builtin_amdgcn_raw_buffer_load_b128(rs, voffj, soff, 0);
      const f32x4 f = __builtin_bit_cast(f32x4, v);
      r[4 * j + 0] = f[0]; r[4 * j + 1] = f[1]; r[4 * j + 2] = f[2]; r[4 * j + 3] = f[3];
    }
  }
};
template <class Cfg>
struct BufShiftedXLoader {
  static constexpr int NCH = Cfg::NCH_B, NREG = NCH * 4;
  const float* base; unsigned ld4; const unsigned* mask;
  unsigned voff[NCH]; int krow[NCH];
  __device__ __forceinline__ void fetch_tile(int kt, float (&r)[NREG]) const {
    const int ku = __builtin_amdgcn_readfirstlane(kt);
    const unsigned w = __builtin_amdgcn_readfirstlane(mask[ku]);
    const __amdgpu_buffer_rsrc_t rs = make_rsrc(base, 0x7fffffffu);
    const unsigned soff = (unsigned)ku * 32u * ld4;
#pragma unroll
    for (int j = 0; j < NCH; ++j) {
      const unsigned voffj = voff[j] | ((__builtin_amdgcn_ubfe(w, (unsigned)krow[j], 1u) ^ 1u) << 31);
      const u32x4 v = __builtin_amdgcn_raw_buffer_load_b128(rs, voffj, soff, 0);
      const f32x4 f = __builtin_bit_cast(f32x4, v);
      r[4 * j + 0] = f[0]; r[4 * j + 1] = f[1]; r[4 * j + 2] = f[2]; r[4 * j + 3] = f[3];
    }
  }
};


constexpr int WGRAD_WIDE_WORDS = 512;
template <class Cfg>
struct BufWideXLoader : BufShiftedXLoader<Cfg> {
  int e0;
  __device__ __forceinline__ int elem(int c) const { return e0 + 8 * (Cfg::BN / 4) * c; }
};

struct XGroup { int s, tap, ci0, kofs, cpad; };
template <int GW>
__device__ __forceinline__ XGroup wgrad_xgroup(const WgradArgs& a, int t, int taps) {
  int s = 0, kofs = 0;
  for (;; ++s) {
    const int ct = (a.src[s].C + GW - 1) / GW;
    if (t < taps * ct) break;
    t -= taps * ct;
    kofs += taps * ((a.src[s].C + 31) / 32) * 32;
  }
  const int C = s == 0 ? a.src[0].C : s == 1 ? a.src[1].C : a.src[2].C;
  const int ct = (C + GW - 1) / GW, cpad = ((C + 31) / 32) * 32;
  const int tap = t / ct, ci0 = (t % ct) * GW;
  return XGroup{s, tap, ci0, kofs + tap * cpad + ci0, cpad};
}

template <class Cfg, bool BUF = false, bool MULTI = false>
__global__ __launch_bounds__(Cfg::NT) void conv_wgrad_split_kernel(const std::conditional_t<MULTI, WgradArgsM, WgradArgs> args) {
  static_assert(Cfg::NT == 256 || BUF, "512-thread workgroups use the buffer-addressed loaders");
  constexpr bool WIDE = Cfg::BN == 256;
  static_assert(!WIDE || (BUF && Cfg::NT == 512), "the 256-column x tile is loaded by two halves of 256 threads");
  constexpr int GW = WIDE ? 128 : Cfg::BN;
  __shared__ __attribute__((aligned(16))) char lds[Cfg::LDS_BYTES];
  __shared__ unsigned pixmask[BUF ? (WIDE ? 2 * WGRAD_WIDE_WORDS : WGRAD_MASK_WORDS) : 1];
  const WgradArgs& a = [&]() -> const WgradArgs& { if constexpr (MULTI) return args.a; else return args; }();
  int bx = blockIdx.x, by = blockIdx.y, zblock = blockIdx.z, seg = 0;
  if (a.xcd_xt > 0) {
    const int span = 8 * a.xcd_xt, r = blockIdx.x / span, rem = blockIdx.x - r * span;
    const int g = r * 8 + (rem & 7);
    if (g >= a.xcd_groups) return;
    if (a.xcd_yt > 0) { bx = rem >> 3; by = g % a.xcd_yt; zblock = g / a.xcd_yt; }
    else { const int tile = rem >> 3, x0 = -a.xcd_yt; bx = tile % x0; by = tile / x0; zblock = g; }
  }
  if constexpr (MULTI) { seg = zblock / args.zs; zblock -= seg * args.zs; seg = __builtin_amdgcn_readfirstlane(seg); }
  bx += a.bx0; by += a.by0;
  const int HW = a.H * a.W;
  const int64_t M = (int64_t)a.B * HW;
  const int taps = a.KH * a.KW;
  const int wave = __builtin_amdgcn_readfirstlane((int)(threadIdx.x >> 6));
  const int xh = WIDE ? wave >> 2 : 0, oh = WIDE ? ((wave % Cfg::WN) * (Cfg::TN * 32)) >> 7 : 0;
  const XGroup gl = wgrad_xgroup<GW>(a, WIDE ? 2 * bx + xh : bx, taps);
  const XGroup go = WIDE ? wgrad_xgroup<GW>(a, 2 * bx + oh, taps) : gl;
  const int s = gl.s;
  Src sc = s == 0 ? a.src[0] : s == 1 ? a.src[1] : a.src[2];
  const float* dyp = a.dy;
  if constexpr (MULTI) {
    typedef const float* fptr;
    const auto* karg = (const char __attribute__((address_space(4)))*)__builtin_amdgcn_kernarg_segment_ptr();
    dyp = ((const fptr __attribute__((address_space(4)))*)(karg + offsetof(WgradArgsM, dys)))[seg];
    sc.p = ((const fptr __attribute__((address_space(4)))*)(karg + offsetof(WgradArgsM, srcs)))[s * WGRAD_MAX_SEG + seg];
  }
  const int tap = gl.tap, ci0 = gl.ci0;
  const int co0 = by * Cfg::BM;
  const int64_t mb = (int64_t)zblock * a.kchunk;
  const int64_t me = mb + a.kchunk < M ? mb + a.kchunk : M;
  if (mb >= M) return;
  const int coleft = ((a.Cout + 3) / 4) * 4 - co0;
  const int cleft = ((sc.C + 3) / 4) * 4 - ci0;
  const int dyy = tap / a.KW - a.KH / 2, dxx = tap % a.KW - a.KW / 2;
  const int KT = (int)((me - mb + 31) / 32);
  f32x16 acc[Cfg::TM][Cfg::TN];
#pragma unroll
  for (int i = 0; i < Cfg::TM; ++i)
#pragma unroll
    for (int j = 0; j < Cfg::TN; ++j)
#pragma unroll
      for (int r = 0; r < 16; ++r) acc[i][j][r] = 0.f;
  float colsum[4] = {0.f, 0.f, 0.f, 0.f};
  const bool want_bias = a.dbias != nullptr && bx == 0;
  if constexpr (BUF) {
    constexpr int MT = WIDE ? 256 : Cfg::NT;
    unsigned* pm = pixmask + xh * WGRAD_WIDE_WORDS;
    for (int i = threadIdx.x % MT; i < KT * 32; i += MT) {
      const int64_t m = mb + i;
      bool ok = m < me;
      if (ok) {
        const int pix = (int)(m % HW), yy = pix / a.W + dyy, xx = pix % a.W + dxx;
        ok = (unsigned)yy < (unsigned)a.H && (unsigned)xx < (unsigned)a.W;
      }
      const unsigned long long bal = __ballot(ok);
      if ((threadIdx.x & 63) == 0) { pm[i >> 5] = (unsigned)bal; pm[(i >> 5) + 1] = (unsigned)(bal >> 32); }
    }
    __syncthreads();
    BufDyLoader<Cfg> la;
    la.base = uni_ptr(dyp + co0 + mb * a.ldy); la.ld4 = uni((unsigned)a.ldy * 4u); la.npix = (int)(me - mb);
    const int cva = coleft < Cfg::BM ? coleft : Cfg::BM;
#pragma unroll
    for (int j = 0; j < BufDyLoader<Cfg>::NCH; ++j) {
      const int e = threadIdx.x + Cfg::NT * j, k = e / (Cfg::BM / 4), c4 = e % (Cfg::BM / 4);
      la.krow[j] = k; la.voff[j] = c4 * 4 < cva ? (unsigned)(k * a.ldy + c4 * 4) * 4u : FS_OOB;
    }
    std::conditional_t<WIDE, BufWideXLoader<Cfg>, BufShiftedXLoader<Cfg>> lb;
    lb.base = uni_ptr(sc.p + ci0 + (mb + dyy * a.W + dxx) * sc.ld); lb.ld4 = uni((unsigned)sc.ld * 4u); lb.mask = pm;
    const int cvb = cleft < GW ? cleft : GW;
    if constexpr (WIDE) {
      const int t8 = threadIdx.x & 255, c4 = t8 & 31;
#pragma unroll
      for (int j = 0; j < BufShiftedXLoader<Cfg>::NCH; ++j) {
        const int k = (t8 >> 5) + 8 * j;
        lb.krow[j] = k; lb.voff[j] = c4 * 4 < cvb ? (unsigned)(k * sc.ld + c4 * 4) * 4u : FS_OOB;
      }
      lb.e0 = (t8 >> 5) * (Cfg::BN / 4) + xh * 32 + c4;
    } else {
#pragma unroll
      for (int j = 0; j < BufShiftedXLoader<Cfg>::NCH; ++j) {
        const int e = threadIdx.x + Cfg::NT * j, k = e / (Cfg::BN / 4), c4 = e % (Cfg::BN / 4);
        lb.krow[j] = k; lb.voff[j] = c4 * 4 < cvb ? (unsigned)(k * sc.ld + c4 * 4) * 4u : FS_OOB;
      }
    }
    if (want_bias) split_mainloop_tn<Cfg, BufDyLoader<Cfg>, decltype(lb), true, WIDE>(lds, KT, la, lb, acc, colsum);
    else split_mainloop_tn<Cfg, BufDyLoader<Cfg>, decltype(lb), false, WIDE>(lds, KT, la, lb, acc);
  } else {
  SplitDyLoader<Cfg> la{dyp + co0, a.ldy, coleft < Cfg::BM ? coleft : Cfg::BM, mb, me};
  SplitShiftedXLoader<Cfg> lb{sc.p + ci0, sc.ld, cleft < Cfg::BN ? cleft : Cfg::BN, dyy, dxx, a.H, a.W, HW, mb, me};
  if (want_bias) split_mainloop_tn<Cfg, SplitDyLoader<Cfg>, SplitShiftedXLoader<Cfg>, true>(lds, KT, la, lb, acc, colsum);
  else split_mainloop_tn<Cfg>(lds, KT, la, lb, acc);
  }
  if (want_bias) {
    constexpr int Q = Cfg::BM / 4, G = Cfg::NT / Q;
    float* part = reinterpret_cast<float*>(lds);
    __syncthreads();
// ... 201 lines not shown

}

#include "wgrad_patch.inc"

namespace {
int g_wgrad_wide = 1;
__thread int t_wgrad_tile = 0;

struct WidePlan {
  int bm;
  int pairs, groups;
  int yw;
  int64_t chunk;
};

WidePlan wide_plan(int Cout, const int* srcC, int nsrc, int taps, int64_t M, int nseg, int64_t chunk128) {
  WidePlan p{};
  if (g_wgrad_wide == 0 || Cout <= 32) return p;
  for (int s = 0; s < nsrc; ++s) p.groups += taps * ceil_div(srcC[s], 128);
  p.pairs = p.groups / 2;
  if (p.pairs == 0) return p;
  const int bm = Cout >= 256 ? 256 : 128;
  const int yw = bm == 256 ? Cout / 256 : ceil_div(Cout, 128);
  const int64_t tiles = (int64_t)p.pairs * yw * nseg, s128 = (M + chunk128 - 1) / chunk128;
  int64_t want = 512 / tiles;
  if (want > s128) want = s128;
  if (tiles * want > 256) want = 256 * (tiles * want / 256) / tiles;
  if (want < 1) want = 1;
  int64_t chunk = (M + want - 1) / want;
  if (chunk < 256) chunk = 256;
  chunk = (chunk + 31) / 32 * 32;
  if (chunk > 32 * (WGRAD_WIDE_WORDS - 2) || chunk * 4 * 2048 >= 0x7fffffff) return p;
  if (g_wgrad_wide == 1) {
    if (tiles * ((M + chunk - 1) / chunk) < 192 || chunk < 512) return p;
  }
  p.bm = bm; p.yw = yw; p.chunk = chunk;
  return p;
}

template <class Cfg, bool MULTI, class A>
int launch_split(A m, int xt, int yt, int zs, int nseg, int bx0, int by0, int64_t chunk, int xcd, hipStream_t stream) {
  WgradArgs& a = [&]() -> WgradArgs& { if constexpr (MULTI) return m.a; else return m; }();
  a.kchunk = (int)chunk; a.bx0 = bx0; a.by0 = by0;
  a.xcd_xt = a.xcd_yt = a.xcd_groups = 0;
  if constexpr (MULTI) { m.zs = zs; m.nseg = nseg; }
  dim3 grid(xt, yt, zs * nseg);
  if (xcd == 3) {
    a.xcd_xt = xt * yt; a.xcd_yt = -xt; a.xcd_groups = zs * nseg;
    grid = dim3((unsigned)(ceil_div(a.xcd_groups, 8) * 8 * xt * yt), 1, 1);
  } else if (xcd) {
    a.xcd_xt = xt; a.xcd_yt = yt; a.xcd_groups = yt * zs * nseg;
    grid = dim3((unsigned)(ceil_div(a.xcd_groups, 8) * 8 * xt), 1, 1);
  }
  hipLaunchKernelGGL((conv_wgrad_split_kernel<Cfg, true, MULTI>), grid, dim3(Cfg::NT), 0, stream, m);
  return fs_launch_status();
}

template <bool MULTI, class A>
int launch_wide(const A& m, const WidePlan& p, int Cout, int64_t M, int nseg, int64_t chunk128, int xcd, hipStream_t stream) {
  const int zsw = (int)((M + p.chunk - 1) / p.chunk), zs = (int)((M + chunk128 - 1) / chunk128);
  int rc = p.bm == 256 ? launch_split<SWCfgW256, MULTI>(m, p.pairs, p.yw, zsw, nseg, 0, 0, p.chunk, xcd, stream)
                       : launch_split<SWCfgW128, MULTI>(m, p.pairs, p.yw, zsw, nseg, 0, 0, p.chunk, xcd, stream);
  if (rc) return rc;
  const int y128 = ceil_div(Cout, 128), ydone = p.bm == 256 ? 2 * p.yw : p.yw;
  if (ydone < y128) rc = launch_split<SWCfg128S, MULTI>(m, p.groups, y128 - ydone, zs, nseg, 0, ydone, chunk128, xcd, stream);
  if (rc) return rc;
  if (p.groups & 1) rc = launch_split<SWCfg128S, MULTI>(m, 1, ydone, zs, nseg, p.groups - 1, 0, chunk128, xcd, stream);
  t_wgrad_tile = p.bm << 16 | 256;
  return rc;
}
}

extern "C" int fsraft_set_wgrad_wide(int mode) {
  if (mode < 0 || mode > 2) return FS_ERR_ARG;
  g_wgrad_wide = mode;
  return FS_OK;
}
extern "C" int fsraft_conv_wgrad_last_tile(void) { return t_wgrad_tile; }

extern "C" int fsraft_conv_wgrad(const float* dy, int ldy, int Cout, const float* const* src, const int* srcC,
                                 const int* srcld, int nsrc, float* dwpk, float* dbias, int B, int H, int W, int KH,
                                 int KW, hipStream_t stream) {
  if (!dy || !src || !dwpk || nsrc < 1 || nsrc > 3 || ldy % 4 != 0) return FS_ERR_ARG;
  t_route[1] = 0; t_wgrad_tile = 0;
  WgradArgs a{};
  a.dy = dy; a.ldy = ldy; a.Cout = Cout;
  const bool small_m = Cout <= 32;
  const bool t64 = !small_m && knob.wgrad_tile == 3;
  const int bn = t64 ? 64 : 128, bm = small_m ? 32 : (t64 ? 64 : 128);
  if (!fill_srcs(a.src, src, srcC, srcld, nsrc)) return FS_ERR_ARG;
  int xt128 = 0;
  for (int s = 0; s < nsrc; ++s) xt128 += KH * KW * ceil_div(srcC[s], bn);
  a.nsrc = nsrc; a.dwpk = dwpk; a.Ktot = conv_ktot(srcC, nsrc, KH * KW);
  a.B = B; a.H = H; a.W = W; a.KH = KH; a.KW = KW;
  const int64_t M = (int64_t)B * H * W;
  if (knob.wgrad_patch && knob.wgrad_patch1 && knob.wgrad_split != 0 && KH == 3 && KW == 3 && Cout > 32 && M >= knob.wgrad_patch1) {
    WgradArgsM m{};
    m.a = a; m.a.dbias = dbias;
    m.nseg = 1;
    m.dys[0] = dy;
    for (int s = 0; s < nsrc; ++s) m.srcs[s][0] = src[s];
    const int rc = launch_wgrad_patch(m, stream);
    if (rc >= 0) return rc;
  }
  if (knob.wgrad_pack && knob.wgrad_split != 0 && knob.wgrad_buf && nsrc == 1 && srcC[0] <= 96 && KH * KW > 1 &&
      (int64_t)(32 * (WGRAD_PACK_WORDS - 2) + 2 * W + 2) * srcld[0] * 4 < 0x7fffffff) {
    const int cpad = ceil_div(srcC[0], 32) * 32;
    int tp = SWCfgPack::BN / cpad;
    if (tp > WGRAD_PACK_SLOTS) tp = WGRAD_PACK_SLOTS;
    const int xt = ceil_div(KH * KW, tp), yt = ceil_div(Cout, SWCfgPack::BM);
    const int64_t chunk = wgrad_chunk(knob.wgrad_blocks_pack, (int64_t)xt * yt, M, WGRAD_PACK_WORDS);
    a.kchunk = (int)chunk;
    a.dbias = dbias;
    dim3 grid(xt, yt, (unsigned)((M + chunk - 1) / chunk));
    if (knob.wgrad_xcd == 2) {
      a.xcd_xt = xt; a.xcd_yt = yt; a.xcd_groups = yt * (int)grid.z;
      grid = dim3((unsigned)(ceil_div(a.xcd_groups, 8) * 8 * xt), 1, 1);
    }
    t_route[1] = 6; t_wgrad_tile = SWCfgPack::BM << 16 | SWCfgPack::BN;
    hipLaunchKernelGGL((conv_wgrad_pack_kernel<SWCfgPack>), grid, dim3(SWCfgPack::NT), 0, stream, a);
    return fs_launch_status();
  }
  const int ytiles = ceil_div(Cout, bm);
  const int64_t chunk = wgrad_chunk(knob.wgrad_blocks, (int64_t)xt128 * ytiles, M, WGRAD_MASK_WORDS);
  a.kchunk = (int)chunk;
  const int zs = (int)((M + chunk - 1) / chunk);
  dim3 grid(xt128, ytiles, zs);
  a.dbias = dbias;
  const bool wbuf = knob.wgrad_buf && chunk <= 32 * (WGRAD_MASK_WORDS - 2) && (int64_t)chunk * 4 * 2048 < 0x7fffffff;
  if (!small_m && !t64 && knob.wgrad_split == 1) {
    t_route[1] = 4; t_wgrad_tile = 128 << 16 | 128;
    if (wbuf) hipLaunchKernelGGL((conv_wgrad_split_kernel<SWCfg128, true>), grid, dim3(256), 0, stream, a);
    else hipLaunchKernelGGL((conv_wgrad_split_kernel<SWCfg128>), grid, dim3(256), 0, stream, a);
    return fs_launch_status();
  }
  if (!small_m && !t64 && knob.wgrad_split == 2) {
    t_route[1] = 5;
    t_wgrad_tile = 128 << 16 | 128;
    if (wbuf) {
      const WidePlan p = wide_plan(Cout, srcC, nsrc, KH * KW, M, 1, chunk);
      if (p.bm) return launch_wide<false>(a, p, Cout, M, 1, chunk, 0, stream);
    }
    if (wbuf)hipLaunchKernelGGL((conv_wgrad_split_kernel<SWCfg128S, true>), grid, dim3(256), 0, stream, a);
    else hipLaunchKernelGGL((conv_wgrad_split_kernel<SWCfg128S>), grid, dim3(256), 0, stream, a);
    return fs_launch_status();
  }
  if (dbias) { const int rc = fsraft_col_sum(dy, ldy, M, Cout, dbias, 1.0f, stream); if (rc) return rc; }
  t_route[1] = small_m ? 1 : t64 ? 2 : 3;
  t_wgrad_tile = bm << 16 | bn;
  if (small_m) hipLaunchKernelGGL((conv_wgrad_kernel<WCfg32>), grid, dim3(256), 0, stream, a);
  else if (t64) hipLaunchKernelGGL((conv_wgrad_kernel<WCfg6464>), grid, dim3(256), 0, stream, a);
  else hipLaunchKernelGGL((conv_wgrad_kernel<WCfg128>), grid, dim3(256), 0, stream, a);
  return fs_launch_status();
}

extern "C" int fsraft_conv_wgrad_multi(const float* const* dy, int nseg, int ldy, int Cout, const float* const* src,
                                       const int* srcC, const int* srcld, int nsrc, float* dwpk, float* dbias, int B,
                                       int H, int W, int KH, int KW, hipStream_t stream) {
  if (!dy || !src || !dwpk || nseg < 1 || nsrc < 1 || nsrc > 3 || ldy % 4 != 0) return FS_ERR_ARG;
  t_route[1] = 0; t_wgrad_tile = 0;
  const int64_t M = (int64_t)B * H * W;
  const bool fast = knob.wgrad_multi && nseg > 1 && Cout > 32 && knob.wgrad_tile != 3 && knob.wgrad_split == 2 && knob.wgrad_buf;
  for (int base = 0; base < nseg; base += WGRAD_MAX_SEG) {
    const int n = nseg - base < WGRAD_MAX_SEG ? nseg - base : WGRAD_MAX_SEG;
    if (!fast || n == 1) {
      for (int i = 0; i < n; ++i) {
        const int rc = fsraft_conv_wgrad(dy[base + i], ldy, Cout, src + (size_t)(base + i) * nsrc, srcC, srcld, nsrc, dwpk,
                                         dbias, B, H, W, KH, KW, stream);
        if (rc) return rc;
// ... 58 lines not shown
```

### flow_supervisor_amd/ops.py

```python
import ctypes
import math
import os

import torch
import torch.optim.optimizer as _optimizer_module

from . import _lib as L


def _lib():
    return L.load()


def parameters_updated(params):
    ps = [p for p in params if isinstance(p, torch.Tensor)]
    if ps:
        torch._C._autograd._unsafe_set_version_counter(ps, [p._version + 1 for p in ps])


def _after_optimizer_step(opt, args, kwargs):
    parameters_updated([p for g in opt.param_groups if g.get("fused") for p in g["params"]])


_optimizer_module.register_optimizer_step_post_hook(_after_optimizer_step)
# ... 1019 lines not shown
            rows, kt = sum(srcC), conv_ktot([cout], kh, kw)
        if frag:
            rows = (rows + 31) // 32 * 32
        j = self._job(ws, cin_full, kh, kw, srcC, srcOff, mode, (1 if frag else 0) | (2 if s2d else 0))
        self.jobs.append((j, self.total, (rows, kt)))
        self.total += (rows * kt + 63) // 64 * 64
        return len(self.jobs) - 1

    def bias(self, bs):
        j = self._job(bs, 1, 1, 1, [1], [0], 3)
        n = sum(b.shape[0] for b in bs)
        self.jobs.append((j, self.total, (n,)))
        self.total += (n + 63) // 64 * 64
        return len(self.jobs) - 1

    def run(self):
        buf = torch.empty(max(self.total, 1), device=self.device, dtype=torch.float32)
        arr = (L.PackJob * max(len(self.jobs), 1))()
        outs = []
        for i, (j, off, shape) in enumerate(self.jobs):
            n = 1
            for v in shape:
                n *= v
            t = buf[off:off + n].view(shape)
            j.wpk = t.data_ptr()
            arr[i] = j
            outs.append(t)
        if self.jobs:
            L.check(_lib().fsraft_pack_conv_weights(arr, len(self.jobs), L.stream()), "pack_conv_weights")
        self.keep = []
        return outs


def unpack_weight_grads(items, device):
    if not items:
        return
    arr = (L.PackJob * len(items))()
    plan = PackPlan(device)
    for i, (dwpk, gs, srcC, srcOff, cin_full, kh, kw, scale, s2d) in enumerate(items):
        j = plan._job(gs, cin_full, kh, kw, srcC, srcOff, 2, 2 if s2d else 0, scale)
        j.wpk = dwpk.data_ptr()
        arr[i] = j
    L.check(_lib().fsraft_pack_conv_weights(arr, len(items), L.stream()), "unpack_conv_weights")


def exact_mode():
    return _lib().fsraft_get_tuning(3) == 0


def set_arithmetic(split):
    global SPLIT_VOLUME_BWD
    L.check(_lib().fsraft_set_arithmetic(1 if split else 0), "set_arithmetic")
    SPLIT_VOLUME_BWD = bool(split)


def pack_pair(w, srcC, dgrad=False):
    m = 1 if dgrad else 0
    split = pack_weight(w, srcC, 10 + m)
    rows = w.shape[1] if dgrad else w.shape[0]
    return (pack_weight(w, srcC, m) if (exact_mode() or rows <= 32) else split), split


def fragment_order(wps):
    N, ktot = wps.shape
    kt, nb = ktot // 32, (N + 31) // 32
    w = wps.contiguous().view(torch.int32)
    if nb * 32 != N:
        w = torch.cat([w, w.new_zeros(nb * 32 - N, ktot)])
    w = w.view(nb, 32, kt, 2, 2, 2, 4).permute(2, 0, 3, 4, 5, 1, 6).contiguous()
    return w.view(torch.float32).view(kt, nb, 4, 64, 4)


def unpack_weight_grad(dwpk, shape, srcC, out=None, accumulate=False):
    Cout, Cin, KH, KW = shape
    if out is None:
        out = torch.empty(shape, device=dwpk.device, dtype=torch.float32)
        accumulate = False
    L.check(_lib().fsraft_pack_conv_weight(L.ptr(out), L.ptr(dwpk), Cout, Cin, KH, KW, L.int_array(srcC), len(srcC), 2,
                                           int(accumulate), L.stream()), "unpack_conv_weight")
    return out


class V:
    __slots__ = ("t", "off", "C", "ld")

    def __init__(self, t, C=None, off=0):
        self.t, self.off, self.ld = t, off, t.shape[-1]
        self.C = (t.shape[-1] - off) if C is None else C
        assert off % 4 == 0 and self.ld % 4 == 0, "channel slices must stay 16-byte aligned"

    @property
    def ptr(self):
        return self.t.data_ptr() + 4 * self.off


class Dst:
    __slots__ = ("t", "off", "bs", "ps", "cs", "n0", "acc", "mask")

    def __init__(self, t, off, bs, ps, cs, n0=0, acc=False):
        self.t, self.off, self.bs, self.ps, self.cs, self.n0, self.acc = t, off, bs, ps, cs, n0, acc
        self.mask = None

    def masked(self, v):
        self.mask = v
        return self

    @staticmethod
    def nhwc(buf, coff=0, n0=0, acc=False):
        B, H, W, ld = buf.shape
        return Dst(buf, coff, H * W * ld, ld, 1, n0, acc)

    @staticmethod
    def nchw(buf, n0=0, acc=False):
        B, C, H, W = buf.shape
        return Dst(buf, 0, C * H * W, 1, H * W, n0, acc)


_CONV_WS = {}
CONV_WS_FLOATS = 24 << 20
CONV_WS_MAX_PIXELS = 16384


def _conv_workspace(device, pixels):
    if pixels > CONV_WS_MAX_PIXELS:
        return None
    key = (torch.device(device).index or 0, torch.cuda.current_stream(device).cuda_stream)
    ws = _CONV_WS.get(key)
    if ws is None:
        ws = _CONV_WS.setdefault(key, torch.empty(CONV_WS_FLOATS, device=device, dtype=torch.float32))
    return ws


def conv_forward(srcs, wpk, bias, B, H, W, KH, KW, N, dsts, relu=False, alpha=1.0, epi=0, h=None, z=None,
                 aux1=None, aux2=None, hid=0, wpk_split=None, pre=None, wpk_frag=None, pad=None, stats=None):
    d = L.ConvDesc()
    for i, v in enumerate(srcs):
        d.src[i] = v.ptr; d.srcC[i] = v.C; d.srcld[i] = v.ld
    d.nsrc = len(srcs)
    d.wpk = wpk.data_ptr()
    d.wpk_split = wpk_split.data_ptr() if wpk_split is not None else None
    d.wpk_frag = wpk_frag.data_ptr() if wpk_frag is not None else None
    if pad is not None:
        d.pad_h1, d.pad_w1 = pad[0] + 1, pad[1] + 1
    d.bias = bias.data_ptr() if bias is not None else None
    d.B, d.H, d.W, d.KH, d.KW, d.N = B, H, W, KH, KW, N
    for i, ds in enumerate(dsts):
        d.dst[i] = ds.t.data_ptr() + 4 * ds.off
        d.dst_bs[i], d.dst_ps[i], d.dst_cs[i] = ds.bs, ds.ps, ds.cs
        d.dst_n0[i] = ds.n0; d.dst_acc[i] = int(ds.acc)
        if ds.mask is not None:
            d.rmask[i] = ds.mask.ptr; d.ldmask[i] = ds.mask.ld; d.maskc[i] = ds.mask.C
    d.ndst = len(dsts)
    d.relu = int(relu); d.alpha = float(alpha); d.epi = epi
    if h is not None:
        d.h = h.data_ptr(); d.ldh = h.shape[-1]
    if z is not None:
        d.z = z.data_ptr(); d.ldz = z.shape[-1]
    if aux1 is not None:
        d.aux1 = aux1.data_ptr(); d.ld1 = aux1.shape[-1]
    if aux2 is not None:
        d.aux2 = aux2.data_ptr(); d.ld2 = aux2.shape[-1]
    d.hid = hid
    if pre is not None:
        d.pre = pre.data_ptr(); d.ldpre = pre.shape[-1]
    ws = _conv_workspace(dsts[0].t.device, B * H * W)
    if ws is not None:
        d.ws = ws.data_ptr(); d.ws_floats = ws.numel()
    t = TIMER
    e0 = t.begin() if t else None
    carried = None
    if stats is not None:
        done = ctypes.c_int(0)
        L.check(_lib().fsraft_conv_forward_stats(ctypes.byref(d), L.ptr(stats[0]), L.ptr(stats[1]), stats.shape[1] // B, ctypes.byref(done),
                                                 L.stream()), "conv_forward_stats")
        carried = bool(done.value)
    else:
        L.check(_lib().fsraft_conv_forward(ctypes.byref(d), L.stream()), "conv_forward")
    if t:
        cin = sum(v.C for v in srcs)
        t.end("conv_igemm", e0, 2.0 * B * H * W * N * cin * KH * KW, 4.0 * B * H * W * (cin + N),
              tag=f"{B}x{H}x{W} {KH}x{KW} {'+'.join(str(v.C) for v in srcs)}->{N} epi{epi}{' relu' if relu else ''}{' masked' if any(ds.mask is not None for ds in dsts) else ''}")
    return carried


def conv_wgrad(dy, srcs, dwpk, B, H, W, KH, KW, dbias=None):
    arr = (ctypes.c_void_p * len(srcs))(*[v.ptr for v in srcs])
    pp = ctypes.cast(arr, L._PP)
    e0w = TIMER.begin() if TIMER else None
    L.check(_lib().fsraft_conv_wgrad(ctypes.c_void_p(dy.ptr), dy.ld, dy.C, pp, L.int_array([v.C for v in srcs]),
                                     L.int_array([v.ld for v in srcs]), len(srcs), L.ptr(dwpk), L.ptr(dbias), B, H, W,
                                     KH, KW, L.stream()), "conv_wgrad")
    if TIMER:
        cin = sum(v.C for v in srcs)
        TIMER.end("conv_wgrad", e0w, 2.0 * B * H * W * dy.C * cin * KH * KW, 4.0 * B * H * W * (cin + dy.C),
                  tag=f"{B}x{H}x{W} {KH}x{KW} {'+'.join(str(v.C) for v in srcs)}->{dy.C} x1")


def conv_wgrad_multi(dys, srcs, dwpk, B, H, W, KH, KW, dbias=None):
    n, nsrc = len(dys), len(srcs[0])
    dy0 = dys[0]
    a_dy = (ctypes.c_void_p * n)(*[v.ptr for v in dys])
    a_src = (ctypes.c_void_p * (n * nsrc))(*[v.ptr for sl in srcs for v in sl])
    e0w = TIMER.begin() if TIMER else None
    L.check(_lib().fsraft_conv_wgrad_multi(ctypes.cast(a_dy, L._PP), n, dy0.ld, dy0.C, ctypes.cast(a_src, L._PP),
                                           L.int_array([v.C for v in srcs[0]]), L.int_array([v.ld for v in srcs[0]]), nsrc,
                                           L.ptr(dwpk), L.ptr(dbias), B, H, W, KH, KW, L.stream()), "conv_wgrad_multi")
    if TIMER:
        cin = sum(v.C for v in srcs[0])
        TIMER.end("conv_wgrad", e0w, 2.0 * n * B * H * W * dy0.C * cin * KH * KW, 4.0 * n * B * H * W * (cin + dy0.C),
                  tag=f"{B}x{H}x{W} {KH}x{KW} {'+'.join(str(v.C) for v in srcs[0])}->{dy0.C} x{n}")


def stem_fwd(x, w, bias=None):
    L.require_cuda_f32(x, w)
    B, C, H, W = x.shape
    N = w.shape[0]
    if C != 3 or tuple(w.shape[1:]) != (3, 7, 7) or not x.is_contiguous():
        raise RuntimeError("stem_fwd: x [B,3,H,W] contiguous and w [N,3,7,7] expected")
    out = torch.empty(B, (H - 1) // 2 + 1, (W - 1) // 2 + 1, N, device=x.device, dtype=torch.float32)
    t = TIMER
    e0 = t.begin() if t else None
    L.check(_lib().fsraft_stem7x7s2_fwd(L.ptr(x), L.ptr(w.contiguous()), L.ptr(bias), L.ptr(out), B, H, W, N, L.stream()), "stem7x7s2_fwd")
    if t:
        t.end("stem", e0, 2.0 * out.numel() * 147, 4.0 * (x.numel() + out.numel()))
    return out


def stem_wgrad(x, dy):
    L.require_cuda_f32(x, dy)
    B, C, H, W = x.shape
    N = dy.shape[-1]
    if not (x.is_contiguous() and dy.is_contiguous()) or tuple(dy.shape[:3]) != (B, (H - 1) // 2 + 1, (W - 1) // 2 + 1):
        raise RuntimeError("stem_wgrad: contiguous x [B,3,H,W] and dy [B,Ho,Wo,N] expected")
    lib = _lib()
    scratch = torch.empty(lib.fsraft_stem_slots() * 64 * 192, device=x.device, dtype=torch.float32)
    dw = torch.empty(N, 3, 7, 7, device=x.device, dtype=torch.float32)
    t = TIMER
    e0 = t.begin() if t else None
    L.check(lib.fsraft_stem7x7s2_wgrad(L.ptr(x), L.ptr(dy), L.ptr(dw), L.ptr(scratch), B, H, W, N, L.stream()), "stem7x7s2_wgrad")
    if t:
        t.end("stem", e0, 2.0 * dy.numel() * 147, 4.0 * (x.numel() + dy.numel()))
    return dw


def conv_small_fwd(x, w_oihw, bias, out_nchw):
    B, N, H, W = out_nchw.shape
    t = TIMER
    e0 = t.begin() if t else None
    L.check(_lib().fsraft_conv_small_fwd(ctypes.c_void_p(x.ptr), x.ld, x.C, L.ptr(w_oihw), L.ptr(bias), L.ptr(out_nchw),
                                         N * H * W, H * W, 1, N, B, H, W, 3, 3, L.stream()), "conv_small_fwd")
    if t:
        t.end("conv_small", e0, 2.0 * B * H * W * N * x.C * 9, 4.0 * B * H * W * (x.C + N))


def conv_small_wgrad(dys, xs, dwpk, dbias, B, H, W):
    n = len(dys)
    a_dy = (ctypes.c_void_p * n)(*[v.ptr for v in dys])
    a_x = (ctypes.c_void_p * n)(*[v.ptr for v in xs])
    L.check(_lib().fsraft_conv_small_wgrad(ctypes.cast(a_dy, L._PP), ctypes.cast(a_x, L._PP), n, dys[0].ld, xs[0].ld, xs[0].C,
                                           L.ptr(dwpk), L.ptr(dbias), dys[0].C, B, H, W, 3, 3, L.stream()), "conv_small_wgrad")


def conv_small_dgrad(dy, w_oihw, dst, mask, B, H, W):
    C = dst.C
    t = TIMER
    e0 = t.begin() if t else None
    L.check(_lib().fsraft_conv_small_dgrad(ctypes.c_void_p(dy.ptr), dy.ld, L.ptr(w_oihw), ctypes.c_void_p(dst.ptr), dst.ld,
                                           ctypes.c_void_p(mask.ptr) if mask is not None else None, mask.ld if mask is not None else 0,
                                           C, 2, B, H, W, 3, 3, L.stream()), "conv_small_dgrad")
    if t:
        t.end("conv_small", e0, 2.0 * B * H * W * 2 * C * 9, 4.0 * B * H * W * (C * (2 if mask is not None else 1) + 2))


def col_sum_v(v, out, scale=1.0):
    M = v.t.numel() // v.ld
    L.check(_lib().fsraft_col_sum(ctypes.c_void_p(v.ptr), v.ld, M, v.C, L.ptr(out), float(scale), L.stream()), "col_sum")

# ... 488 lines not shown
```

### include/fsraft.h

```cpp
#ifndef FSRAFT_H
#define FSRAFT_H

#include <stdint.h>

#ifdef __cplusplus
extern "C" {
#endif

#ifndef __HIP_PLATFORM_AMD__
typedef struct ihipStream_t* hipStream_t;
#endif

#define FSRAFT_OK 0
#define FSRAFT_ERR_ARG 1
#define FSRAFT_ERR_LAUNCH 2

int fsraft_corr_build(const float* fmap1, const float* fmap2, float* const* levels, int num_levels,
                      int B, int C, int H, int W, hipStream_t stream);

int fsraft_corr_pool_pyramid(float* const* levels, int num_levels, int64_t rows, int H2, int W2, hipStream_t stream);
int fsraft_corr_pool_pyramid_same(float* const* levels, int num_levels, int64_t rows, int H2, int W2, hipStream_t stream);
int fsraft_corr_lookup_fwd_same(float* const* levels, int num_levels, const float* coords, int64_t coords_bs,
                                int64_t coords_cs, int64_t coords_ps, float* out, int nhwc_out, int B, int H, int W,
                                int radius, hipStream_t stream);
int fsraft_corr_unpool_bwd(float* const* dlevels, int num_levels, int B, int H, int W, hipStream_t stream);
int fsraft_corr_unpool_same_bwd(float* const* dlevels, int num_levels, int64_t rows, int H2, int W2, hipStream_t stream);
int fsraft_corr_lookup_bwd_same(float* const* dlevels, int num_levels, const float* coords, int64_t coords_bs,
                                int64_t coords_cs, int64_t coords_ps, const float* dout, int nhwc_in, int B, int H, int W,
                                int radius, hipStream_t stream);
int fsraft_corr_lookup_dcoords_same(float* const* levels, int num_levels, const float* coords, int64_t coords_bs, int64_t coords_cs,
                                    int64_t coords_ps, const float* dout, int nhwc_in, float* dcoords, int64_t dbs, int64_t dcs,
                                    int64_t dps, int B, int H, int W, int radius, hipStream_t stream);

int fsraft_vol_layout(int H, int W, int num_levels, int* out);
int fsraft_corr_build_tiled(const float* fmap1, const float* fmap2, float* vol, int num_levels, int B, int C, int H, int W,
                            hipStream_t stream);
int fsraft_corr_build_rec(const void* f1r, const void* f2r, float* vol, int num_levels, int B, int C, int H, int W,
                          hipStream_t stream);
int fsraft_corr_lookup_tiled_fwd(const float* vol, int num_levels, const float* coords, int64_t coords_bs, int64_t coords_cs,
                                 int64_t coords_ps, float* out, int B, int H, int W, int radius, int add_grid, hipStream_t stream);
int fsraft_corr_lookup_tiled_dcoords(const float* vol, int num_levels, const float* coords, int64_t coords_bs, int64_t coords_cs,
                                     int64_t coords_ps, const float* dout, float* dcoords, int64_t dbs, int64_t dcs, int64_t dps,
                                     int B, int H, int W, int radius, int add_grid, hipStream_t stream);
int fsraft_corr_dvol_build(const float* const* dout, const float* const* coords, const int64_t* coords_str, int n, float* dvol,
                           int num_levels, int B, int H, int W, int radius, int accumulate, int records, int add_grid,
                           int64_t q0, int64_t nq, unsigned* qlist, const unsigned* wmask,
                           hipStream_t stream);
int fsraft_corr_f2cat(const float* fmap2, float* f2cat, int num_levels, int B, int C, int H, int W, hipStream_t stream);
int fsraft_corr_dfmap2(const float* d2cat, float* d2, int num_levels, int B, int C, int H, int W, hipStream_t stream);
int fsraft_corr_f2cat_rec(const float* fmap2, void* f2r, int num_levels, int B, int C, int H, int W, hipStream_t stream);

int fsraft_corr_lookup_fwd(float* const* levels, int num_levels, const float* coords, int64_t coords_bs,
                           int64_t coords_cs, int64_t coords_ps, float* out, int nhwc_out, int B, int H, int W,
                           int radius, hipStream_t stream);
int fsraft_corr_lookup_bwd(float* const* dlevels, int num_levels, const float* coords, int64_t coords_bs,
                           int64_t coords_cs, int64_t coords_ps, const float* dout, int nhwc_in, int B, int H, int W,
                           int radius, hipStream_t stream);
int fsraft_corr_lookup_dcoords(float* const* levels, int num_levels, const float* coords, int64_t coords_bs, int64_t coords_cs,
                               int64_t coords_ps, const float* dout, int nhwc_in, float* dcoords, int64_t dbs, int64_t dcs,
                               int64_t dps, int B, int H, int W, int radius, hipStream_t stream);

int fsraft_altcorr_fwd(const float* fmap1, const float* fmap2, const float* coords, float* corr, int B, int N, int H1,
                       int W1, int H2, int W2, int C, int radius, hipStream_t stream);
int fsraft_altcorr_bwd(const float* fmap1, const float* fmap2, const float* coords, const float* corr_grad,
                       float* fmap1_grad, float* fmap2_grad, int B, int N, int H1, int W1, int H2, int W2, int C,
                       int radius, hipStream_t stream);

int fsraft_altcorr_fused_fwd(const float* fmap1, const float* const* fmap2_levels, int num_levels, const float* coords,
                             int64_t coords_bs, int64_t coords_cs, int64_t coords_ps, int add_grid, float* out, int B, int H, int W,
                             int C, int radius, hipStream_t stream);
int fsraft_altcorr_fused_dcoords(const float* fmap1, const float* const* fmap2_levels, int num_levels, const float* coords,
                                 int64_t coords_bs, int64_t coords_cs, int64_t coords_ps, int add_grid, const float* dout,
                                 float* dcoords, int64_t dbs, int64_t dcs, int64_t dps, int B, int H, int W, int C, int radius,
                                 hipStream_t stream);

int fsraft_altcorr_mfma_fwd(const void* f1r, const void* const* f2r_levels, const float* fmap1, const float* const* fmap2_levels,
                            int num_levels, const float* coords, int64_t coords_bs, int64_t coords_cs, int64_t coords_ps,
                            int add_grid, float* out, int B, int H, int W, int C, int radius, hipStream_t stream);

int fsraft_upsample_fwd(const float* flow, int64_t flow_bs, int64_t flow_cs, int64_t flow_ps,
                        const float* mask_nhwc, float* up, int N, int H, int W, hipStream_t stream);
int fsraft_upsample_bwd(const float* flow, int64_t flow_bs, int64_t flow_cs, int64_t flow_ps,
                        const float* mask_nhwc, const float* dup, float* dmask_nhwc, float* dflow, float* scratch,
                        int N, int H, int W, hipStream_t stream);
int fsraft_upflow8_fwd(const float* flow, float* up, int N, int C, int H, int W, hipStream_t stream);
int fsraft_upflow8_bwd(const float* dup, float* dflow, int N, int C, int H, int W, hipStream_t stream);

typedef struct fsraft_conv_desc {
  const float* src[3]; int srcC[3]; int srcld[3]; int nsrc;
  const float* wpk; const float* bias;
  const float* wpk_split;
  int B, H, W, KH, KW, N;
  float* dst[3]; int64_t dst_bs[3]; int64_t dst_ps[3]; int64_t dst_cs[3];
  int dst_n0[3]; int dst_acc[3]; int ndst;
  int relu; float alpha;
  int epi;
  const float* h; int ldh; const float* z; int ldz;
  float* aux1; int ld1; float* aux2; int ld2; int hid;
  const float* pre; int ldpre;
  const float* rmask[3]; int ldmask[3]; int maskc[3];
  const float* wpk_frag;
  int pad_h1, pad_w1;
  float* ws; int64_t ws_floats;
} fsraft_conv_desc;

int fsraft_conv_ktot(const int* srcC, int nsrc, int KH, int KW);
int fsraft_conv_forward(const fsraft_conv_desc* d, hipStream_t stream);
int fsraft_conv_forward_stats(const fsraft_conv_desc* d, float* sum, float* sq, int slots, int* done, hipStream_t stream);
int fsraft_conv_wgrad(const float* dy, int ldy, int Cout, const float* const* src, const int* srcC,
                      const int* srcld, int nsrc, float* dwpk, float* dbias, int B, int H, int W, int KH, int KW,
                      hipStream_t stream);
int fsraft_conv_wgrad_multi(const float* const* dy, int nseg, int ldy, int Cout, const float* const* src,
                            const int* srcC, const int* srcld, int nsrc, float* dwpk, float* dbias, int B, int H, int W,
                            int KH, int KW, hipStream_t stream);
int fsraft_pack_conv_weight(float* w_oihw, float* wpk, int Cout, int Cin, int KH, int KW, const int* srcC,
                            int nsrc, int mode, int accumulate, hipStream_t stream);

typedef struct {
  float* w[3]; int rows[3]; int npiece;
  float* wpk;
  int cin_full, kh, kw;
  int srcC[3], srcOff[3], nsrc;
  int mode, flags;
  float scale; int accumulate;
} fsraft_pack_job;
int fsraft_pack_conv_weights(const fsraft_pack_job* jobs, int njobs, hipStream_t stream);

int fsraft_conv_small_fwd(const float* x, int ld, int C, const float* w_oihw, const float* bias, float* out, int64_t obs,
                          int64_t ocs, int64_t ops, int N, int B, int H, int W, int KH, int KW, hipStream_t stream);
int fsraft_conv_small_wgrad(const float* const* dy, const float* const* x, int nseg, int ldy, int ldx, int C, float* dwpk,
                            float* dbias, int N, int B, int H, int W, int KH, int KW, hipStream_t stream);
int fsraft_conv_small_dgrad(const float* dy, int ldy, const float* w_oihw, float* dx, int lddx, const float* relu_src, int ldm,
                            int C, int N, int B, int H, int W, int KH, int KW, hipStream_t stream);

int fsraft_conv_workspace(float* ws, int64_t floats);

int fsraft_set_arithmetic(int mode);
int fsraft_get_arithmetic(void);

int fsraft_gemm_f32(const float* A, int64_t lda, int64_t sA, const float* Bm, int64_t ldb, int64_t sB, float* C,
                    int64_t ldc, int64_t sC, int batch, int M, int N, int K, int trans_b, float alpha,
                    int accumulate, hipStream_t stream);

int fsraft_gemm_tn_split(const float* A, int64_t lda, int64_t sA, const float* Bm, int64_t ldb, int64_t sB, float* C,
                         int64_t ldc, int64_t sC, int batch, int M, int N, int K, float alpha, int accumulate,
                         hipStream_t stream);

int fsraft_to_records(const float* src, int64_t ld, void* dst, int64_t dst_ld, int64_t rows, int K, hipStream_t stream);
int fsraft_gemm_rec_nt(const void* A, int64_t lda, int64_t sA, const void* Bm, int64_t ldb, int64_t sB, float* C, int64_t ldc,
                       int64_t sC, int batch, int M, int N, int K, float alpha, int ksplit, int accumulate, hipStream_t stream);
int fsraft_gemm_rec_tn(const void* A, int64_t lda, int64_t sA, const void* Bm, int64_t ldb, int64_t sB, float* C, int64_t ldc,
                       int64_t sC, int batch, int M, int N, int K, float alpha, int ksplit, int accumulate, hipStream_t stream);

int fsraft_gemm_rec_nt_list(const void* A, int64_t lda, int64_t sA, const void* Bm, int64_t ldb, int64_t sB, float* C, int64_t ldc,
                            int64_t sC, int batch, int M, int N, int K, float alpha, int ksplit, int accumulate, const int* klist,
                            const int* kcount, int kl_stride, int kl_by_n, hipStream_t stream);
int fsraft_gemm_rec_tn_list(const void* A, int64_t lda, int64_t sA, const void* Bm, int64_t ldb, int64_t sB, float* C, int64_t ldc,
                            int64_t sC, int batch, int M, int N, int K, float alpha, int ksplit, int accumulate, const int* klist,
                            const int* kcount, int kl_stride, int kl_by_n, hipStream_t stream);
int fsraft_corr_bwd_ktiles(const float* const* coords, const int64_t* coords_str, int n, int num_levels, int B, int H, int W,
                           int radius, int add_grid, int64_t q0, int64_t nq, int* nt_list, int* nt_count, int nt_stride, unsigned* tn_bits,
                           int* tn_list, int* tn_count, int tn_stride, unsigned* wmask, hipStream_t stream);

int fsraft_softmax_rows(float* S, int64_t rows, int n, hipStream_t stream);
int fsraft_softmax_rows_bwd(const float* A, float* dA, int64_t rows, int n, hipStream_t stream);
int fsraft_softmax_rows_rec(float* S, int64_t rows, int n, hipStream_t stream);
int fsraft_softmax_rows_bwd_rec(const void* A_records, float* dA, int64_t rows, int n, hipStream_t stream);
int fsraft_softmax_rows_pos(float* S, const float* G, int64_t ldg, int64_t rows, int n, int h, int w, int content, int records,
                            hipStream_t stream);
int fsraft_softmax_rows_pos_bwd(const void* A, float* dA, float* dG, int64_t ldg, int64_t rows, int n, int h, int w, int records,
                                hipStream_t stream);
int fsraft_gma_mix_fwd(const float* x, int ldx, const float* y, int ldy, const float* gamma, float* dst, int ldd,
                       int64_t M, int C, hipStream_t stream);
int fsraft_gma_mix_bwd(const float* d, int ldd, const float* y, int ldy, const float* gamma, float* dx, int ldx,
                       float* dy, int lddy, float* dgamma, int64_t M, int C, hipStream_t stream);

int fsraft_inorm_relu_fwd(const float* x, float* y, float* stats, int64_t planes, int HW, float eps, int relu, hipStream_t stream);
int fsraft_inorm_relu_bwd(const float* g, const float* x, const float* stats, float* dx, int64_t planes, int HW, int relu,
                          hipStream_t stream);
int fsraft_affine_relu_fwd(const float* x, const float* scale, const float* shift, float* y, int64_t planes, int C, int HW,
                           int relu, hipStream_t stream);
int fsraft_affine_relu_bwd(const float* g, const float* x, const float* scale, const float* shift, float* dx, float* dsum_g,
                           float* dsum_gx, int64_t planes, int C, int HW, int relu, hipStream_t stream);

int fsraft_sequence_loss(const float* const* pred, float* const* dpred, const float* weights, int n, int metric_idx,
                         const float* gt, const float* valid, float max_flow, float eps, int B, int H, int W, float* out,
                         hipStream_t stream);

#define FSRAFT_FLOW_L1 0
#define FSRAFT_FLOW_L2 1
#define FSRAFT_FLOW_ROBUST 2
int fsraft_flow_loss_workspace_bytes(int B, int H, int W);
int fsraft_flow_loss(const float* const* pred, float* const* dpred, const float* weights, int n,
                     int64_t pred_bs, int64_t pred_cs, int64_t pred_ps,
// ... 134 lines not shown
```

### include/fsraft_tuning.h

```cpp
#ifndef FSRAFT_TUNING_H
#define FSRAFT_TUNING_H

#ifdef __cplusplus
extern "C" {
#endif

enum fsraft_tuning_key {
  FSRAFT_KEY_CONV_TILE = 0,
  FSRAFT_KEY_WGRAD_TILE = 1,
  FSRAFT_KEY_WGRAD_BLOCKS = 2,
  FSRAFT_KEY_CONV_ARITH = 3,
  FSRAFT_KEY_WGRAD_ARITH = 4,
  FSRAFT_KEY_CONV_BUF = 5,
  FSRAFT_KEY_XCD_SWIZZLE = 7,
  FSRAFT_KEY_WGRAD_BUF = 8,
  FSRAFT_KEY_CONV_N256 = 9,
  FSRAFT_KEY_WGRAD_MULTI = 10,
  FSRAFT_KEY_WGRAD_BLOCKS_MULTI = 11,
  FSRAFT_KEY_CONV_UNIFORM = 12,
  FSRAFT_KEY_CONV_W8 = 13,
  FSRAFT_KEY_CONV_W8_MIN = 14,
  FSRAFT_KEY_WGRAD_W8 = 15,
  FSRAFT_KEY_WGRAD_PACK = 16,
  FSRAFT_KEY_WGRAD_BLOCKS_PACK = 17,
  FSRAFT_KEY_CONV_N64 = 18,
  FSRAFT_KEY_CONV_N64_MIN_M = 19,
  FSRAFT_KEY_CONV_HALO = 20,
  FSRAFT_KEY_CONV_HALO_MIN_M = 21,
  FSRAFT_KEY_WGRAD_XCD = 22,
  FSRAFT_KEY_CONV_PATCH = 26,
  FSRAFT_KEY_WGRAD_PATCH = 27,
  FSRAFT_KEY_CONV_PATCH64 = 28,
  FSRAFT_KEY_WGRAD_PATCH1 = 29,
  FSRAFT_KEY_CONV_PATCH_MIN_M = 31,
  FSRAFT_KEY_CONV_KSPLIT = 32
};
int fsraft_set_tuning(int key, int value);
int fsraft_get_tuning(int key);
int fsraft_conv_last_route(int which);
int fsraft_set_wgrad_wide(int mode);
int fsraft_conv_wgrad_last_tile(void);
int fsraft_set_build_split(int on);
int fsraft_set_build_kernel(int which);
int fsraft_set_lookup_policy(int aux);
int fsraft_set_ktile_exact(int levels);
int fsraft_set_upsample_kernel(int v4);
int fsraft_set_dvol_box(int on);
int fsraft_set_dvol_policy(int policy);
int fsraft_set_gemm_split(int on);
int fsraft_set_lookup_qb(int qb);
int fsraft_set_norm_blocks(int target_workgroups);
int fsraft_set_rec_mfma16(int on);
int fsraft_set_alt_tile(int on);

#ifdef __cplusplus
}
#endif
#endif
```

Baseline: 115.7 image-pairs/s.

## Skip structurally-zero k-tiles in space-to-depth stride-2 conv fwd and wgrad

```diff
diff --git a/flow_supervisor_amd/_lib.py b/flow_supervisor_amd/_lib.py
--- a/flow_supervisor_amd/_lib.py
+++ b/flow_supervisor_amd/_lib.py
@@ -27,6 +27,7 @@
         ("rmask", c_void_p * 3), ("ldmask", c_int * 3), ("maskc", c_int * 3),
         ("wpk_frag", c_void_p), ("pad_h1", c_int), ("pad_w1", c_int),
         ("ws", c_void_p), ("ws_floats", c_int64),
+        ("s2d_c", c_int),
     ]
 
 
@@ -72,6 +73,7 @@
     "fsraft_conv_forward": [POINTER(ConvDesc), _S],
     "fsraft_conv_forward_stats": [POINTER(ConvDesc), c_void_p, c_void_p, c_int, POINTER(c_int), _S],
     "fsraft_conv_wgrad": [c_void_p, c_int, c_int, _PP, _IP, _IP, c_int, c_void_p, c_void_p, c_int, c_int, c_int, c_int, c_int, _S],
+    "fsraft_conv_wgrad_s2d": [c_void_p, c_int, c_int, _PP, _IP, _IP, c_int, c_void_p, c_void_p, c_int, c_int, c_int, c_int, c_int, c_int, _S],
     "fsraft_conv_wgrad_multi": [_PP, c_int, c_int, c_int, _PP, _IP, _IP, c_int, c_void_p, c_void_p, c_int, c_int, c_int, c_int, c_int, _S],
     "fsraft_conv_small_fwd": [c_void_p, c_int, c_int, c_void_p, c_void_p, c_void_p, c_int64, c_int64, c_int64, c_int, c_int, c_int, c_int, c_int, c_int, _S],
     "fsraft_conv_small_wgrad": [_PP, _PP, c_int, c_int, c_int, c_int, c_void_p, c_void_p, c_int, c_int, c_int, c_int, c_int, c_int, _S],
@@ -138,6 +140,7 @@
     "fsraft_get_tuning": [c_int],
     "fsraft_conv_last_route": [c_int],
     "fsraft_set_wgrad_wide": [c_int],
+    "fsraft_set_s2d_live": [c_int],
     "fsraft_conv_wgrad_last_tile": [],
     "fsraft_space_to_depth2": [c_void_p, c_void_p, c_int, c_int, c_int, c_int, c_int, _S],
     "fsraft_forward_interpolate": [c_void_p, c_void_p, c_int, c_int, _S],
diff --git a/flow_supervisor_amd/core/extractor.py b/flow_supervisor_amd/core/extractor.py
--- a/flow_supervisor_amd/core/extractor.py
+++ b/flow_supervisor_amd/core/extractor.py
@@ -415,7 +415,7 @@
         y1 = torch.empty(B, h, w, N, device=x.device, dtype=torch.float32)
         ys = torch.empty(B, h, w, Ns, device=x.device, dtype=torch.float32)
         p, q = packs.conv3, packs.shortcut
-        ops.conv_forward([ops.V(xs, 4 * C)], p.fwd, None, B, h, w, 2, 2, N, [ops.Dst.nhwc(y1)], wpk_split=p.fwd_split)
+        ops.conv_forward([ops.V(xs, 4 * C, s2d_c=C)], p.fwd, None, B, h, w, 2, 2, N, [ops.Dst.nhwc(y1)], wpk_split=p.fwd_split)
         ops.conv_forward([ops.V(xs, C, 0)], q.fwd, None, B, h, w, 1, 1, Ns, [ops.Dst.nhwc(ys)], wpk_split=q.fwd_split)
         ctx.save_for_backward(xs, w3, wsc)
         ctx.packs = packs
@@ -438,7 +438,7 @@
         items = []
         if ctx.needs_input_grad[1]:
             dwpk = ops.zeros(N, ops.conv_ktot([C4], 2, 2), device=xs.device)
-            ops.conv_wgrad(g1v, [ops.V(xs, C4)], dwpk, B, h, w, 2, 2)
+            ops.conv_wgrad(g1v, [ops.V(xs, C4, s2d_c=C)], dwpk, B, h, w, 2, 2)
             dw3 = torch.empty(N, C, 3, 3, device=xs.device, dtype=torch.float32)
             items.append((dwpk, [dw3], [C4], [0], C, 2, 2, 1.0, True))
         if ctx.needs_input_grad[2]:
diff --git a/flow_supervisor_amd/csrc/conv_common.hpp b/flow_supervisor_amd/csrc/conv_common.hpp
--- a/flow_supervisor_amd/csrc/conv_common.hpp
+++ b/flow_supervisor_amd/csrc/conv_common.hpp
@@ -34,6 +34,7 @@
   int wgrad_patch1 = 8192;
   int conv_patch_min_m = 8192;
   int conv_ksplit = -1;
+  int s2d_live = 1;
 };
 __attribute__((visibility("hidden"))) extern ConvKnobs knob;
 __attribute__((visibility("hidden"))) extern __thread int t_route[2];
@@ -60,14 +61,21 @@
   float* st_sum; float* st_sq; int st_slots;
   int swz;
   int ksplit;
+  int s2d_c;
 };
 
+__host__ __device__ inline bool s2d_slot_live(int tap, int sub) { return (((tap >> 1) | (sub >> 1)) & ((tap & 1) | (sub & 1))) != 0; }
+
 constexpr int KTAB_MAX = 512;
+constexpr int KSPLIT_MAX = 6;
 struct ConvArgsT {
   ConvArgs a;
   const float* ubase; int uld;
+  int kts;
   unsigned ktab[KTAB_MAX];
+  unsigned kstart[KSPLIT_MAX + 2];
 };
+static_assert(sizeof(ConvArgsT) <= 4096, "the table travels in the kernarg segment");
 
 enum { EPI_PLAIN = 0, EPI_ZR = 2, EPI_Q = 3 };
 
diff --git a/flow_supervisor_amd/csrc/conv_igemm.hip b/flow_supervisor_amd/csrc/conv_igemm.hip
--- a/flow_supervisor_amd/csrc/conv_igemm.hip
+++ b/flow_supervisor_amd/csrc/conv_igemm.hip
@@ -78,7 +78,7 @@
   }
 };
 
-template <class Cfg>
+template <class Cfg, bool WT = false>
 struct BufConvALoader {
   static constexpr int NCH = Cfg::NCH_A, NREG = NCH * 4;
   const float* b0; const float* b1; const float* b2; unsigned nb0, nb1, nb2;
@@ -89,7 +89,7 @@
   unsigned kq16;
   __device__ __forceinline__ void fetch_tile(int kt, float (&r)[NREG]) const {
     const unsigned e = ktab[__builtin_amdgcn_readfirstlane(kt)];
-    const unsigned soff = (e & 0xffffu) << 4, tap = (e >> 16) & 15u, src = (e >> 20) & 3u, crem = (e >> 22) & 63u;
+    const unsigned soff = (e & 0xffffu) << 4, tap = (e >> 16) & 15u, src = WT ? 0u : (e >> 20) & 3u, crem = WT ? 32u : (e >> 22) & 63u;
     const bool s1 = src >= 1, s2 = src >= 2;
     const unsigned ldb = ld0x4 + (s1 ? ld1x4 - ld0x4 : 0u) + (s2 ? ld2x4 - ld1x4 : 0u);
     const float* bp = b0 + (s1 ? b1 - b0 : 0) + (s2 ? b2 - b1 : 0);
@@ -109,7 +109,7 @@
   }
 };
 
-template <class Cfg>
+template <class Cfg, bool WT = false>
 struct BufConvALoaderU {
   static constexpr int NCH = Cfg::NCH_A, NREG = NCH * 4;
   const float* base;
@@ -120,7 +120,7 @@
   __device__ __forceinline__ void fetch_tile(int kt, float (&r)[NREG]) const {
     const int ku = __builtin_amdgcn_readfirstlane(kt);
     const unsigned soff = ktab[2 * ku], e = ktab[2 * ku + 1];
-    const unsigned tap = e & 15u, crem4 = (e >> 4) * 4u;
+    const unsigned tap = e & 15u, crem4 = (WT ? (e >> 4) & 63u : e >> 4) * 4u;
     const __amdgpu_buffer_rsrc_t rs = make_rsrc(base, 0x7fffffffu);
     const unsigned cok = kq16 < crem4 ? 1u : 0u;
 #pragma unroll
@@ -136,15 +136,19 @@
   }
 };
 
-template <class Cfg>
+template <class Cfg, int WT = 0>
 struct BufWeightLoader {
   static constexpr int NCH = Cfg::NCH_B, NREG = NCH * 4;
   const char* base; unsigned nbytes;
+  const unsigned __attribute__((address_space(4)))* ktab;
   unsigned voff[NCH];
   __device__ __forceinline__ void fetch_tile(int kt, float (&r)[NREG]) const {
     const int ku = __builtin_amdgcn_readfirstlane(kt);
     const __amdgpu_buffer_rsrc_t rs = make_rsrc(base, ku < 0 ? 0u : nbytes);
-    const unsigned soff = ku < 0 ? 0u : (unsigned)ku * 128u;
+    unsigned wt = ku < 0 ? 0u : (unsigned)ku;
+    if constexpr (WT == 1) wt = ktab[wt] >> 20;
+    if constexpr (WT == 2) wt = ktab[2 * wt + 1] >> 16;
+    const unsigned soff = wt * 128u;
 #pragma unroll
     for (int j = 0; j < NCH; ++j) {
       const u32x4 v = __builtin_amdgcn_raw_buffer_load_b128(rs, voff[j], soff, 0);
@@ -479,9 +483,10 @@
   conv_epilogue<Cfg, EPI>(a, acc, m0, n0);
 }
 
-template <class Cfg, int EPI, int BUF = 0>
+template <class Cfg, int EPI, int BUF = 0, bool WT = false>
 __global__ __launch_bounds__(Cfg::NT) void conv_igemm_split_kernel(const std::conditional_t<BUF != 0, ConvArgsT, ConvArgs> args) {
   static_assert(Cfg::NT == 256 || BUF != 0, "wider workgroups use the buffer-addressed loaders");
+  static_assert(!WT || BUF != 0, "the live form is a form of the k-tile table");
   __shared__ __attribute__((aligned(16))) char lds[Cfg::LDS_ALLOC];
   const ConvArgs& a = [&]() -> const ConvArgs& { if constexpr (BUF != 0) return args.a; else return args; }();
   const int HW = a.H * a.W;
@@ -501,7 +506,17 @@
     const auto* ktab = (const unsigned __attribute__((address_space(4)))*)(
         (const char __attribute__((address_space(4)))*)__builtin_amdgcn_kernarg_segment_ptr() + offsetof(ConvArgsT, ktab));
     int kt0 = 0, KTs = a.Ktot / 32;
-    if (a.ksplit > 1) {
+    if constexpr (WT) {
+      KTs = args.kts;
+      if (a.ksplit > 1) {
+        const auto* kstart = (const unsigned __attribute__((address_space(4)))*)(
+            (const char __attribute__((address_space(4)))*)__builtin_amdgcn_kernarg_segment_ptr() + offsetof(ConvArgsT, kstart));
+        const int z = __builtin_amdgcn_readfirstlane((int)blockIdx.z);
+        kt0 = (int)kstart[z];
+        KTs = (int)kstart[z + 1] - kt0;
+        ktab += kt0 * (BUF >= 2 ? 2 : 1);
+      }
+    } else if (a.ksplit > 1) {
       const int per = (KTs + a.ksplit - 1) / a.ksplit;
       kt0 = (int)blockIdx.z * per;
       KTs = min(per, KTs - kt0);
@@ -521,23 +536,24 @@
       }
       tapmask[j] = mask; pofs[j] = m < M ? m : 0;
     }
-    BufWeightLoader<Cfg> lb;
-    lb.base = uni_ptr(reinterpret_cast<const char*>(a.wpk) + (int64_t)n0 * a.Ktot * 4 + (int64_t)kt0 * 128);
+    BufWeightLoader<Cfg, WT ? BUF : 0> lb;
+    lb.base = uni_ptr(reinterpret_cast<const char*>(a.wpk) + (int64_t)n0 * a.Ktot * 4 + (WT ? (int64_t)0 : (int64_t)kt0 * 128));
+    lb.ktab = ktab;
     lb.nbytes = 0x7fffffffu;
 #pragma unroll
-    for (int j = 0; j < BufWeightLoader<Cfg>::NCH; ++j) {
+    for (int j = 0; j < Cfg::NCH_B; ++j) {
       const int e = threadIdx.x + Cfg::NT * j;
       lb.voff[j] = (e >> 3) < a.N - n0 ? (unsigned)((e >> 3) * a.Ktot * 4 + (e & 7) * 16) : FS_OOB;
     }
     if constexpr (BUF >= 2) {
-      BufConvALoaderU<Cfg> la;
+      BufConvALoaderU<Cfg, WT> la;
       la.base = uni_ptr(args.ubase); la.ktab = ktab; la.kq16 = (threadIdx.x & 7) * 16;
       const unsigned ldb = uni((unsigned)args.uld * 4u);
 #pragma unroll
       for (int j = 0; j < Cfg::NCH_A; ++j) { la.tapmask[j] = tapmask[j]; la.voff0[j] = pofs[j] * ldb + la.kq16; }
-      split_mainloop<Cfg, BufConvALoaderU<Cfg>, BufWeightLoader<Cfg>, true>(lds, KTs, la, lb, acc);
+      split_mainloop<Cfg, decltype(la), decltype(lb), true>(lds, KTs, la, lb, acc);
     } else {
-      BufConvALoader<Cfg> la;
+      BufConvALoader<Cfg, WT> la;
       la.ld0x4 = uni(a.src[0].ld * 4); la.ld1x4 = uni(a.src[1].ld * 4); la.ld2x4 = uni(a.src[2].ld * 4);
       la.b0 = uni_ptr(a.src[0].p - (int64_t)(PH * a.W + PW) * a.src[0].ld); la.nb0 = 0x7fffffffu;
       la.b1 = uni_ptr(a.src[1].p - (int64_t)(PH * a.W + PW) * a.src[1].ld); la.nb1 = 0x7fffffffu;
@@ -546,7 +562,7 @@
       la.kq16 = (threadIdx.x & 7) * 16;
 #pragma unroll
       for (int j = 0; j < Cfg::NCH_A; ++j) { la.tapmask[j] = tapmask[j]; la.pofs[j] = pofs[j]; }
-      split_mainloop<Cfg, BufConvALoader<Cfg>, BufWeightLoader<Cfg>, true>(lds, KTs, la, lb, acc);
+      split_mainloop<Cfg, decltype(la), decltype(lb), true>(lds, KTs, la, lb, acc);
     }
     if constexpr (EPI == EPI_PLAIN && Cfg::LDS_ALLOC >= Cfg::BM * (Cfg::BN + 4) * 4) {
       if (a.ksplit > 1) {
@@ -753,31 +769,38 @@
   return fs_launch_status();
 }
 
-bool build_ktab(const ConvArgs& a, ConvArgsT& t) {
+bool build_ktab(const ConvArgs& a, ConvArgsT& t, bool live = false, int slices = 1) {
   const int taps = a.KH * a.KW, KT = a.Ktot / 32;
   const int64_t M = (int64_t)a.B * a.H * a.W;
-  if (KT > KTAB_MAX || taps > 15) return false;
-  int kt = 0;
+  if (KT > KTAB_MAX || taps > 15 || (live && slices > KSPLIT_MAX)) return false;
+  const int per = (KT + slices - 1) / slices;
+  int kt = 0, n = 0;
   for (int s = 0; s < a.nsrc; ++s) {
     const int C = a.src[s].C, ld = a.src[s].ld, cpt = (C + 31) / 32;
     if (M * ld * 4 >= (int64_t)FS_OOB) return false;
     for (int i = 0; i < taps * cpt; ++i, ++kt) {
         const int tap = i / cpt, c = i % cpt;
+        if (live && kt % per == 0) t.kstart[kt / per] = (unsigned)n;
+        if (live && !s2d_slot_live(tap, c * 32 / a.s2d_c)) continue;
         const int64_t soff = ((int64_t)((tap / a.KW) * a.W + tap % a.KW) * ld + c * 32) * 4;
         if (soff % 16 != 0 || soff / 16 > 0xffff) return false;
         const int crem = C - c * 32 < 32 ? C - c * 32 : 32;
-        t.ktab[kt] = (unsigned)(soff / 16) | (unsigned)tap << 16 | (unsigned)s << 20 | (unsigned)crem << 22;
+        t.ktab[n++] = live ? (unsigned)(soff / 16) | (unsigned)tap << 16 | (unsigned)kt << 20
+                           : (unsigned)(soff / 16) | (unsigned)tap << 16 | (unsigned)s << 20 | (unsigned)crem << 22;
       }
   }
   if (kt != KT) return false;
-  t.a = a;
+  if (live) for (int z = (KT + per - 1) / per; z <= KSPLIT_MAX + 1; ++z) t.kstart[z] = (unsigned)n;
+  t.a = a; t.kts = n;
   return true;
 }
 
-bool build_ktab_uniform(const ConvArgs& a, ConvArgsT& t) {
+bool build_ktab_uniform(const ConvArgs& a, ConvArgsT& t, bool live = false, int slices = 1) {
   const int taps = a.KH * a.KW, KT = a.Ktot / 32, PH = a.PH, PW = a.PW;
   const int64_t M = (int64_t)a.B * a.H * a.W;
-  if (!knob.conv_uniform || 2 * KT > KTAB_MAX || taps > 15) return false;
+  if (!knob.conv_uniform || 2 * KT > KTAB_MAX || taps > 15 || (live && slices > KSPLIT_MAX)) return false;
+  const int per = (KT + slices - 1) / slices;
+  int n = 0;
   const int ld = a.src[0].ld;
   const float* lo = a.src[0].p;
   for (int s = 0; s < a.nsrc; ++s) {
@@ -791,16 +814,25 @@
     const int64_t delta = (a.src[s].p - lo) * 4;
     for (int tap = 0; tap < taps; ++tap)
       for (int c = 0; c < cpt; ++c, ++kt) {
+        if (live && kt % per == 0) t.kstart[kt / per] = (unsigned)n;
+        if (live && !s2d_slot_live(tap, c * 32 / a.s2d_c)) continue;
         const int64_t soff = delta + ((int64_t)((tap / a.KW) * a.W + tap % a.KW) * ld + c * 32) * 4;
         if (soff + M * ld * 4 + 256 >= (int64_t)FS_OOB) return false;
         const int crem = C - c * 32 < 32 ? C - c * 32 : 32;
-        t.ktab[2 * kt] = (unsigned)soff;
-        t.ktab[2 * kt + 1] = (unsigned)tap | (unsigned)crem << 4;
+        t.ktab[2 * n] = (unsigned)soff;
+        t.ktab[2 * n + 1] = (unsigned)tap | (unsigned)crem << 4 | (live ? (unsigned)kt << 16 : 0u);
+        ++n;
       }
   }
   if (kt != KT) return false;
-  t.a = a; t.ubase = base; t.uld = ld;
+  if (live) for (int z = (KT + per - 1) / per; z <= KSPLIT_MAX + 1; ++z) t.kstart[z] = (unsigned)n;
+  t.a = a; t.ubase = base; t.uld = ld; t.kts = n;
   return true;
+}
+
+bool s2d_live_ok(const ConvArgs& a, int epi) {
+  return knob.s2d_live && a.s2d_c > 0 && a.s2d_c % 32 == 0 && epi == EPI_PLAIN && a.KH == 2 && a.KW == 2 && a.PH == 1 && a.PW == 1 &&
+         a.nsrc == 1 && a.src[0].C == 4 * a.s2d_c;
 }
 
 
@@ -904,13 +936,15 @@
   ConvArgsT t;
   const int swz = knob.xcd_swizzle || (grid.x >= 2 && (int64_t)grid.x * grid.y >= 2048);
   const bool buf = knob.conv_buf == 2 || (knob.conv_buf == 1 && Cfg::BM == 64) || Cfg::BN == 256 || Cfg::NT != 256;
+  const bool live = buf && s2d_live_ok(a, epi);
   if constexpr (Cfg::LDS_ALLOC >= Cfg::BM * (Cfg::BN + 4) * 4) {
     const int ldw = (a.N + 3) / 4 * 4;
     const bool gru_ok = epi == EPI_PLAIN || (a.N % 4 == 0 && (!a.pre || a.ldpre % 4 == 0));
     const int S = (buf && g_conv_ws && gru_ok && (Cfg::BM == 64 || (Cfg::BM == 128 && Cfg::NT == 512) || knob.conv_ksplit >= 2)) ? pick_ksplit((int64_t)grid.x * grid.y, a.Ktot / 32, a.N, M, ldw, Cfg::BM) : 1;
     if (S > 1) {
-      const bool uni_tab = build_ktab_uniform(a, t);
-      if (uni_tab || build_ktab(a, t)) {
+      const bool lv = live && S <= KSPLIT_MAX;
+      const bool uni_tab = build_ktab_uniform(a, t, lv, S);
+      if (uni_tab || build_ktab(a, t, lv, S)) {
         ConvArgs& p = t.a;
         p.swz = 0;
         p.ksplit = S;
@@ -920,7 +954,9 @@
         for (int i = 0; i < 3; ++i) p.rmask[i] = nullptr;
         dim3 g3(grid.x, grid.y, S);
         t_route[0] = route_split<Cfg>() + 100;
-        if (uni_tab) hipLaunchKernelGGL((conv_igemm_split_kernel<Cfg, EPI_PLAIN, 2>), g3, dim3(Cfg::NT), 0, s, t);
+        if (lv && uni_tab) hipLaunchKernelGGL((conv_igemm_split_kernel<Cfg, EPI_PLAIN, 2, true>), g3, dim3(Cfg::NT), 0, s, t);
+        else if (lv) hipLaunchKernelGGL((conv_igemm_split_kernel<Cfg, EPI_PLAIN, 1, true>), g3, dim3(Cfg::NT), 0, s, t);
+        else if (uni_tab) hipLaunchKernelGGL((conv_igemm_split_kernel<Cfg, EPI_PLAIN, 2>), g3, dim3(Cfg::NT), 0, s, t);
         else hipLaunchKernelGGL((conv_igemm_split_kernel<Cfg, EPI_PLAIN, 1>), g3, dim3(Cfg::NT), 0, s, t);
         int rc = fs_launch_status();
         if (rc) return rc;
@@ -930,6 +966,18 @@
         return fs_launch_status();
       }
     }
+  }
+  if (live && build_ktab_uniform(a, t, true)) {
+    t.a.swz = swz;
+    t_route[0] = route_split<Cfg>();
+    hipLaunchKernelGGL((conv_igemm_split_kernel<Cfg, EPI_PLAIN, 2, true>), grid, dim3(Cfg::NT), 0, s, t);
+    return fs_launch_status();
+  }
+  if (live && build_ktab(a, t, true)) {
+    t.a.swz = swz;
+    t_route[0] = route_split<Cfg>();
+    hipLaunchKernelGGL((conv_igemm_split_kernel<Cfg, EPI_PLAIN, 1, true>), grid, dim3(Cfg::NT), 0, s, t);
+    return fs_launch_status();
   }
   if (buf && build_ktab_uniform(a, t)) {
     t.a.swz = swz;
@@ -1002,6 +1050,7 @@
   const bool want_stats = t_stat.sum != nullptr && d->epi == EPI_PLAIN && d->ndst == 1 && !d->relu && d->alpha == 1.0f && !d->dst_acc[0] &&
                           !d->rmask[0] && !d->bias && d->dst_n0[0] == 0 && d->N % 4 == 0;
   if (d->ws && (((uintptr_t)d->ws & 15) || d->ws_floats < 0)) return FS_ERR_ARG;
+  if (d->s2d_c < 0) return FS_ERR_ARG;
   t_route[0] = 0;
   g_conv_ws = d->ws ? d->ws : t_reg_ws;
   g_conv_ws_floats = d->ws ? d->ws_floats : t_reg_ws_floats;
@@ -1057,6 +1106,7 @@
   const int M = d->B * d->H * d->W;
   if (knob.conv_split && d->wpk_split && d->N > 32) {
     a.wpk = d->wpk_split;
+    a.s2d_c = knob.conv_split == 1 ? d->s2d_c : 0;
     const bool narrow = knob.conv_buf != 0 || (int64_t)ceil_div(d->N, 128) * ceil_div(M, 128) < 400;
     if (knob.conv_patch && knob.conv_split == 1 && d->KH * d->KW > 1 && d->N > 64 && M >= knob.conv_patch_min_m) {
       ConvArgs p = a;
diff --git a/flow_supervisor_amd/csrc/conv_tuning.hip b/flow_supervisor_amd/csrc/conv_tuning.hip
--- a/flow_supervisor_amd/csrc/conv_tuning.hip
+++ b/flow_supervisor_amd/csrc/conv_tuning.hip
@@ -55,6 +55,12 @@
   return k ? *k : INT_MIN;
 }
 
+extern "C" int fsraft_set_s2d_live(int on) {
+  if (on != 0 && on != 1) return FS_ERR_ARG;
+  knob.s2d_live = on;
+  return FS_OK;
+}
+
 extern "C" int fsraft_conv_last_route(int which) {
   return which == 0 || which == 1 ? t_route[which] : -1;
 }
diff --git a/flow_supervisor_amd/csrc/conv_wgrad.hip b/flow_supervisor_amd/csrc/conv_wgrad.hip
--- a/flow_supervisor_amd/csrc/conv_wgrad.hip
+++ b/flow_supervisor_amd/csrc/conv_wgrad.hip
@@ -11,6 +11,7 @@
   float* dbias;
   int xcd_xt, xcd_yt, xcd_groups;
   int bx0, by0;
+  int s2d_c;
 };
 
 constexpr int WGRAD_MAX_SEG = 16;
@@ -173,6 +174,16 @@
   return XGroup{s, tap, ci0, kofs + tap * cpad + ci0, cpad};
 }
 
+template <int GW>
+__device__ __forceinline__ bool wgrad_group_dead(const WgradArgs& a, int t) {
+  const int C4 = a.src[0].C, ct = (C4 + GW - 1) / GW;
+  const int tap = t / ct, ci0 = (t % ct) * GW, ci1 = min(ci0 + GW, C4) - 1;
+  if (tap >= a.KH * a.KW) return false;
+  for (int sub = ci0 / a.s2d_c; sub <= ci1 / a.s2d_c; ++sub)
+    if (s2d_slot_live(tap, sub)) return false;
+  return true;
+}
+
 template <class Cfg, bool BUF = false, bool MULTI = false>
 __global__ __launch_bounds__(Cfg::NT) void conv_wgrad_split_kernel(const std::conditional_t<MULTI, WgradArgsM, WgradArgs> args) {
   static_assert(Cfg::NT == 256 || BUF, "512-thread workgroups use the buffer-addressed loaders");
@@ -195,6 +206,10 @@
   const int HW = a.H * a.W;
   const int64_t M = (int64_t)a.B * HW;
   const int taps = a.KH * a.KW;
+  if (a.s2d_c > 0 && !(a.dbias != nullptr && bx == 0)) {
+    const bool dead = WIDE ? wgrad_group_dead<GW>(a, 2 * bx) && wgrad_group_dead<GW>(a, 2 * bx + 1) : wgrad_group_dead<GW>(a, bx);
+    if (dead) return;
+  }
   const int wave = __builtin_amdgcn_readfirstlane((int)(threadIdx.x >> 6));
   const int xh = WIDE ? wave >> 2 : 0, oh = WIDE ? ((wave % Cfg::WN) * (Cfg::TN * 32)) >> 7 : 0;
   const XGroup gl = wgrad_xgroup<GW>(a, WIDE ? 2 * bx + xh : bx, taps);
@@ -562,10 +577,17 @@
 extern "C" int fsraft_conv_wgrad(const float* dy, int ldy, int Cout, const float* const* src, const int* srcC,
                                  const int* srcld, int nsrc, float* dwpk, float* dbias, int B, int H, int W, int KH,
                                  int KW, hipStream_t stream) {
-  if (!dy || !src || !dwpk || nsrc < 1 || nsrc > 3 || ldy % 4 != 0) return FS_ERR_ARG;
+  return fsraft_conv_wgrad_s2d(dy, ldy, Cout, src, srcC, srcld, nsrc, dwpk, dbias, B, H, W, KH, KW, 0, stream);
+}
+
+extern "C" int fsraft_conv_wgrad_s2d(const float* dy, int ldy, int Cout, const float* const* src, const int* srcC,
+                                     const int* srcld, int nsrc, float* dwpk, float* dbias, int B, int H, int W, int KH,
+                                     int KW, int s2d_c, hipStream_t stream) {
+  if (!dy || !src || !dwpk || nsrc < 1 || nsrc > 3 || ldy % 4 != 0 || s2d_c < 0) return FS_ERR_ARG;
   t_route[1] = 0; t_wgrad_tile = 0;
   WgradArgs a{};
   a.dy = dy; a.ldy = ldy; a.Cout = Cout;
+  a.s2d_c = (knob.s2d_live && s2d_c > 0 && s2d_c % 32 == 0 && KH == 2 && KW == 2 && nsrc == 1 && srcC[0] == 4 * s2d_c) ? s2d_c : 0;
   const bool small_m = Cout <= 32;
   const bool t64 = !small_m && knob.wgrad_tile == 3;
   const int bn = t64 ? 64 : 128, bm = small_m ? 32 : (t64 ? 64 : 128);
diff --git a/flow_supervisor_amd/ops.py b/flow_supervisor_amd/ops.py
--- a/flow_supervisor_amd/ops.py
+++ b/flow_supervisor_amd/ops.py
@@ -1125,10 +1125,10 @@
 
 
 class V:
-    __slots__ = ("t", "off", "C", "ld")
-
-    def __init__(self, t, C=None, off=0):
-        self.t, self.off, self.ld = t, off, t.shape[-1]
+    __slots__ = ("t", "off", "C", "ld", "s2d_c")
+
+    def __init__(self, t, C=None, off=0, s2d_c=0):
+        self.t, self.off, self.ld, self.s2d_c = t, off, t.shape[-1], s2d_c
         self.C = (t.shape[-1] - off) if C is None else C
         assert off % 4 == 0 and self.ld % 4 == 0, "channel slices must stay 16-byte aligned"
 
@@ -1177,6 +1177,8 @@
 def conv_forward(srcs, wpk, bias, B, H, W, KH, KW, N, dsts, relu=False, alpha=1.0, epi=0, h=None, z=None,
                  aux1=None, aux2=None, hid=0, wpk_split=None, pre=None, wpk_frag=None, pad=None, stats=None):
     d = L.ConvDesc()
+    s2d_c = srcs[0].s2d_c if len(srcs) == 1 else 0
+    d.s2d_c = s2d_c
     for i, v in enumerate(srcs):
         d.src[i] = v.ptr; d.srcC[i] = v.C; d.srcld[i] = v.ld
     d.nsrc = len(srcs)
@@ -1221,21 +1223,28 @@
         L.check(_lib().fsraft_conv_forward(ctypes.byref(d), L.stream()), "conv_forward")
     if t:
         cin = sum(v.C for v in srcs)
-        t.end("conv_igemm", e0, 2.0 * B * H * W * N * cin * KH * KW, 4.0 * B * H * W * (cin + N),
+        t.end("conv_igemm", e0, 2.0 * B * H * W * N * _live_products(cin, KH, KW, s2d_c), 4.0 * B * H * W * (cin + N),
               tag=f"{B}x{H}x{W} {KH}x{KW} {'+'.join(str(v.C) for v in srcs)}->{N} epi{epi}{' relu' if relu else ''}{' masked' if any(ds.mask is not None for ds in dsts) else ''}")
     return carried
 
 
+def _live_products(cin, KH, KW, s2d_c):
+    if s2d_c and (KH, KW) == (2, 2) and cin == 4 * s2d_c:
+        return 9 * s2d_c
+    return cin * KH * KW
+
+
 def conv_wgrad(dy, srcs, dwpk, B, H, W, KH, KW, dbias=None):
+    s2d_c = srcs[0].s2d_c if len(srcs) == 1 else 0
     arr = (ctypes.c_void_p * len(srcs))(*[v.ptr for v in srcs])
     pp = ctypes.cast(arr, L._PP)
     e0w = TIMER.begin() if TIMER else None
-    L.check(_lib().fsraft_conv_wgrad(ctypes.c_void_p(dy.ptr), dy.ld, dy.C, pp, L.int_array([v.C for v in srcs]),
-                                     L.int_array([v.ld for v in srcs]), len(srcs), L.ptr(dwpk), L.ptr(dbias), B, H, W,
-                                     KH, KW, L.stream()), "conv_wgrad")
+    L.check(_lib().fsraft_conv_wgrad_s2d(ctypes.c_void_p(dy.ptr), dy.ld, dy.C, pp, L.int_array([v.C for v in srcs]),
+                                         L.int_array([v.ld for v in srcs]), len(srcs), L.ptr(dwpk), L.ptr(dbias), B, H, W,
+                                         KH, KW, s2d_c, L.stream()), "conv_wgrad")
     if TIMER:
         cin = sum(v.C for v in srcs)
-        TIMER.end("conv_wgrad", e0w, 2.0 * B * H * W * dy.C * cin * KH * KW, 4.0 * B * H * W * (cin + dy.C),
+        TIMER.end("conv_wgrad", e0w, 2.0 * B * H * W * dy.C * _live_products(cin, KH, KW, s2d_c), 4.0 * B * H * W * (cin + dy.C),
                   tag=f"{B}x{H}x{W} {KH}x{KW} {'+'.join(str(v.C) for v in srcs)}->{dy.C} x1")
 
 
diff --git a/include/fsraft.h b/include/fsraft.h
--- a/include/fsraft.h
+++ b/include/fsraft.h
@@ -102,6 +102,7 @@
   const float* wpk_frag;
   int pad_h1, pad_w1;
   float* ws; int64_t ws_floats;
+  int s2d_c;
 } fsraft_conv_desc;
 
 int fsraft_conv_ktot(const int* srcC, int nsrc, int KH, int KW);
@@ -110,6 +111,9 @@
 int fsraft_conv_wgrad(const float* dy, int ldy, int Cout, const float* const* src, const int* srcC,
                       const int* srcld, int nsrc, float* dwpk, float* dbias, int B, int H, int W, int KH, int KW,
                       hipStream_t stream);
+int fsraft_conv_wgrad_s2d(const float* dy, int ldy, int Cout, const float* const* src, const int* srcC,
+                          const int* srcld, int nsrc, float* dwpk, float* dbias, int B, int H, int W, int KH, int KW,
+                          int s2d_c, hipStream_t stream);
 int fsraft_conv_wgrad_multi(const float* const* dy, int nseg, int ldy, int Cout, const float* const* src,
                             const int* srcC, const int* srcld, int nsrc, float* dwpk, float* dbias, int B, int H, int W,
                             int KH, int KW, hipStream_t stream);
diff --git a/include/fsraft_tuning.h b/include/fsraft_tuning.h
--- a/include/fsraft_tuning.h
+++ b/include/fsraft_tuning.h
@@ -40,6 +40,7 @@
 int fsraft_conv_last_route(int which);
 int fsraft_set_wgrad_wide(int mode);
 int fsraft_conv_wgrad_last_tile(void);
+int fsraft_set_s2d_live(int on);
 int fsraft_set_build_split(int on);
 int fsraft_set_build_kernel(int which);
 int fsraft_set_lookup_policy(int aux);
```

Result: no change. 116.0 image-pairs/s (median of 6 runs) (+0.3%).
